# Zain-Jiang/Dict-TTS

Measured on AMD Instinct MI355X. Metric: mel-frames/sec, end-to-end text->mel->wav (audio-samples/sec = 256x; RTF reported alongside), higher is better.
Workload: dtype f16 (vocoder ResBlocks fp16 MFMA, serial convolutions bf16 hi/lo split; acoustic model fp32-grade: fp32 MFMA / bf16 three-piece operands x 6 products)

## Files before the change

dict_tts_amd/csrc/context.hip:

```cpp
#include "ctx.h"

using namespace dtts;

constexpr int TUNE_RELEASE_MASK = (1 << 8) | (1 << 9) | (1 << 12) | (1 << 13) | (1 << 14) | (1 << 15);

static std::string g_create_err;

namespace dtts {

int fail(dtts_ctx* h, int code, const char* fmt, ...) {
    char buf[512];
    va_list ap;
    va_start(ap, fmt);
    vsnprintf(buf, sizeof buf, fmt, ap);
    va_end(ap);
    if (h) h->err = buf;
    else g_create_err = buf;
    return code;
}

}

extern "C" {

int dtts_config_sizeof(void) { return (int)sizeof(dtts_config); }

void dtts_default_config(dtts_config* c) {
    memset(c, 0, sizeof *c);
    c->hidden_size = 192;
    c->num_heads = 2;
    c->enc_ffn_kernel_size = 5;
    c->enc_layers = 4;
    c->gloss_dim = 768;
    c->word_size = 8000;
    c->value_embedding_size = 185;
    c->n_phone = 6;
    c->audio_num_mel_bins = 80;
    c->latent_size = 16;
    c->fvae_enc_dec_hidden = 192;
    c->fvae_kernel_size = 5;
    c->fvae_dec_n_layers = 4;
    c->fvae_enc_n_layers = 8;
    c->prior_glow_hidden = 64;
    c->glow_kernel_size = 3;
    c->prior_glow_n_blocks = 4;
    c->prior_glow_n_layers = 4;
    c->dur_predictor_layers = 3;
    c->dur_predictor_kernel = 5;
    c->dur_chans = 128;
    c->frames_multiple = 4;
    c->language_zh = 1;
    c->upsample_initial_channel = 512;
    c->n_upsamples = 4;
    const int ur[4] = {8, 8, 2, 2}, uk[4] = {16, 16, 4, 4}, rk[3] = {3, 7, 11};
    for (int i = 0; i < 4; ++i) {
        c->upsample_rates[i] = ur[i];
        c->upsample_kernel_sizes[i] = uk[i];
    }
    c->n_resblock_kernels = 3;
    for (int i = 0; i < 3; ++i) {
        c->resblock_kernel_sizes[i] = rk[i];
        c->resblock_dilation_sizes[i][0] = 1;
        c->resblock_dilation_sizes[i][1] = 3;
        c->resblock_dilation_sizes[i][2] = 5;
    }
    c->vocoder_precision = DTTS_VOC_F16;
    c->fft_layers = 4;
    c->fft_kernel_size = 9;
    c->fft_use_pos_embed = 1;
    c->fft_use_last_norm = 1;
}

int dtts_create(const dtts_config* cfg, dtts_handle* out) {
    if (!cfg || !out) return fail(nullptr, DTTS_E_INVAL, "dtts_create: null argument");
    if (cfg->tune_flags & ~TUNE_RELEASE_MASK)
        return fail(nullptr, DTTS_E_INVAL, "dtts_create: tune_flags 0x%x carries bits this library does not honour (supported mask 0x%x)",
                    (unsigned)cfg->tune_flags, (unsigned)TUNE_RELEASE_MASK);
    if (cfg->n_resblock_kernels >= 0 && cfg->n_resblock_kernels <= 4) {
        int two = 0;
        for (int j = 0; j < cfg->n_resblock_kernels; ++j) {
            const int32_t* d = cfg->resblock_dilation_sizes[j];
            if (d[0] < 1 || d[1] < 1 || d[2] < 0)
                return fail(nullptr, DTTS_E_INVAL, "dtts_create: resblock_dilation_sizes[%d] = (%d, %d, %d): the first two dilations must be >= 1, the third >= 1 (ResBlock1) or 0 (ResBlock2)",
                            j, (int)d[0], (int)d[1], (int)d[2]);
            two += d[2] == 0 ? 1 : 0;
        }
        if (two != 0 && two != cfg->n_resblock_kernels)
            return fail(nullptr, DTTS_E_INVAL, "dtts_create: resblock_dilation_sizes mixes two-dilation (ResBlock2, third entry 0) and three-dilation (ResBlock1) rows: "
                        "%d of %d rows have a third entry of 0", two, (int)cfg->n_resblock_kernels);
    }
    int ndev = 0;
    if (hipGetDeviceCount(&ndev) != hipSuccess || ndev == 0)
        return fail(nullptr, DTTS_E_HIP, "dtts_create: no HIP device visible (the HIP path has no CPU fallback)");
    if (cfg->hidden_size % 64 || cfg->hidden_size / cfg->num_heads > 96 || cfg->gloss_dim > 768 || cfg->gloss_dim % 4 ||
        cfg->n_upsamples > 8 || cfg->n_resblock_kernels > 4 || cfg->latent_size % 8 || cfg->prior_glow_hidden % 32 ||
        cfg->fvae_enc_dec_hidden % 32)
        return fail(nullptr, DTTS_E_INVAL, "dtts_create: unsupported configuration");
    dtts_ctx* h = new dtts_ctx();
    h->cfg = *cfg;
    h->tune = cfg->tune_flags;
    {
        static unsigned long long instance = 0;
        int dev = 0;
        (void)hipGetDevice(&dev);
        unsigned long long z = (unsigned long long)time(nullptr) * 0x9E3779B97F4A7C15ull ^ ((unsigned long long)getpid() << 32) ^
                               ((unsigned long long)dev << 20) ^ ++instance;
        z = (z ^ (z >> 30)) * 0xBF58476D1CE4E5B9ull;
        z = (z ^ (z >> 27)) * 0x94D049BB133111EBull;
        h->noise_seed = z ^ (z >> 31);
    }
    h->guard_on = cfg->vocoder_range_guard != 0;
    h->resblock2 = cfg->n_resblock_kernels > 0 && cfg->resblock_dilation_sizes[0][2] == 0;
    (void)hipGetDevice(&h->device);
    if (hipDeviceGetAttribute(&h->n_cu, hipDeviceAttributeMultiprocessorCount, h->device) != hipSuccess || h->n_cu <= 0) h->n_cu = 256;
    h->debug_rz = cfg->debug_redzone != 0;
    h->a_fft.debug = h->a_enc.debug = h->a_dec.debug = h->a_voc.debug = h->a_spk.debug = h->a_post.debug = h->debug_rz;
    *out = h;
    return DTTS_OK;
}

void dtts_destroy(dtts_handle h) {
    if (h && h->bad_host) {
        (void)hipDeviceSynchronize();
        (void)hipHostFree((void*)h->bad_host);
        h->bad_host = nullptr;
    }
    if (!h) return;
    (void)hipDeviceSynchronize();
    for (void* p : h->allocs) (void)hipFree(p);
    if (h->amax_bits) (void)hipFree(h->amax_bits);
    h->a_fft.release();
    h->a_enc.release();
    h->a_dec.release();
    h->a_voc.release();
    h->a_spk.release();
    h->a_post.release();
    for (auto& t : h->timers)
        for (auto e : t.pool) (void)hipEventDestroy(e);
    delete h;
}

const char* dtts_last_error(dtts_handle h) { return h ? h->err.c_str() : g_create_err.c_str(); }

int dtts_load_weight(dtts_handle h, const char* name, const void* host_ptr, const int64_t* shape, int ndim, int dtype) {
    if (!h || !name || !host_ptr || ndim < 0 || ndim > 8) return fail(h, DTTS_E_INVAL, "dtts_load_weight: bad argument");
    if (dtype != DTTS_F32) return fail(h, DTTS_E_INVAL, "dtts_load_weight(%s): only fp32 tensors are accepted", name);
    HostTensor t;
    t.shape.assign(shape, shape + ndim);
    const int64_t n = t.numel();
    t.f.assign((const float*)host_ptr, (const float*)host_ptr + n);
    h->w[name] = std::move(t);
    return DTTS_OK;
}

int dtts_finalize_weights(dtts_handle h, int parts) {
    if (!h) return DTTS_E_INVAL;
    h->err.clear();
    int rc = DTTS_OK;
    if ((parts & DTTS_PART_ACOUSTIC) && !h->acoustic_ready) rc = build_acoustic(h);
    if (rc == DTTS_OK && (parts & DTTS_PART_VOCODER) && !h->vocoder_ready) rc = build_vocoder(h);
    if (rc == DTTS_OK && (parts & DTTS_PART_FFT) && !h->fft_ready) rc = build_fft(h);
    if (rc == DTTS_OK) {
        for (auto it = h->w.begin(); it != h->w.end();) {
            const bool a = it->first.rfind("model.", 0) == 0 && h->acoustic_ready;
            const bool v = it->first.rfind("vocoder.", 0) == 0 && h->vocoder_ready;
            const bool f = it->first.rfind("fft.", 0) == 0 && h->fft_ready;
            it = (a || v || f) ? h->w.erase(it) : std::next(it);
        }
    }
    return rc;
}

int dtts_load_weights(dtts_handle h, const char* name, const void* host_ptr, const int64_t* shape, int ndim, int dtype) {
    return dtts_load_weight(h, name, host_ptr, shape, ndim, dtype);
}

int dtts_timer_enable(dtts_handle h, int which) {
    if (!h || which < 1 || which >= DTTS_TIMER_COUNT) return DTTS_E_INVAL;
    h->timers[which].enabled = true;
    return DTTS_OK;
}

static void timer_collect(TimerSlot& t) {
    for (size_t i = 0; i + 1 < t.used; i += 2) {
        float ms = 0;
        if (hipEventElapsedTime(&ms, t.pool[i], t.pool[i + 1]) == hipSuccess) t.ms_done += ms;
    }
    t.used = 0;
}

int dtts_timer_read(dtts_handle h, int which, double* ms_total, int64_t* launches) {
    if (!h || which < 1 || which >= DTTS_TIMER_COUNT) return DTTS_E_INVAL;
    HIPCHK(hipDeviceSynchronize());
    TimerSlot& t = h->timers[which];
    timer_collect(t);
    if (ms_total) *ms_total = t.ms_done;
    if (launches) *launches = t.launches;
    return DTTS_OK;
}

int dtts_timer_reset(dtts_handle h) {
    if (!h) return DTTS_E_INVAL;
    HIPCHK(hipDeviceSynchronize());
    for (auto& t : h->timers) {
        t.used = 0;
        t.ms_done = 0;
        t.launches = 0;
    }
    return DTTS_OK;
}

namespace {
struct RzZone { const unsigned char* p; unsigned n; unsigned id; };
__global__ void redzone_check_kernel(const RzZone* z, int nz, unsigned long long* out) {
    const RzZone q = z[blockIdx.x];
    unsigned bad = 0;
    for (unsigned i = threadIdx.x; i < q.n; i += blockDim.x) bad += q.p[i] != 0xFF ? 1u : 0u;
    if (bad) {
        atomicAdd(out, (unsigned long long)bad);
        atomicMin(out + 1, (unsigned long long)q.id);
    }
}
}

int dtts_debug_poke(dtts_handle h, dtts_stream stream) {
    if (!h) return DTTS_E_INVAL;
    if (!h->debug_rz) return fail(h, DTTS_E_STATE, "dtts_debug_poke: the context was not created with dtts_config.debug_redzone = 1");
    char* target = nullptr;
    for (Arena* a : {&h->a_voc, &h->a_enc, &h->a_dec, &h->a_fft, &h->a_spk, &h->a_post})
        if (!target && a->base && !a->bufs.empty()) target = a->base + a->bufs[0].start + a->bufs[0].bytes;
    if (!target && !h->rz_static.empty()) target = h->rz_static[0].p + h->rz_static[0].bytes;
    if (!target) return fail(h, DTTS_E_STATE, "dtts_debug_poke: nothing allocated yet");
    HIPCHK(hipMemsetAsync(target, 0, 1, (hipStream_t)stream));
    return DTTS_OK;
}

int dtts_debug_check(dtts_handle h, int64_t* damaged_bytes, dtts_stream stream) {
    if (!h || !damaged_bytes) return DTTS_E_INVAL;
    *damaged_bytes = -1;
    if (!h->debug_rz) return fail(h, DTTS_E_STATE, "dtts_debug_check: the context was not created with dtts_config.debug_redzone = 1");
    hipStream_t s = (hipStream_t)stream;
    HIPCHK(hipStreamSynchronize(s));
    std::vector<RzZone> zones;
    std::vector<std::string> names;
    auto zone = [&](const char* p0, size_t n, const std::string& name) {
        if (!n) return;
        zones.push_back({(const unsigned char*)p0, (unsigned)n, (unsigned)names.size()});
        names.push_back(name);
    };
    const std::pair<const char*, Arena*> arenas[] = {{"encode workspace", &h->a_enc}, {"decode workspace", &h->a_dec}, {"vocoder workspace", &h->a_voc}, {"fft workspace", &h->a_fft}, {"speaker workspace", &h->a_spk}, {"posterior workspace", &h->a_post}};
    for (const auto& a : arenas) {
        const auto& bufs = a.second->bufs;
        const char* base = a.second->base;
        for (size_t i = 0; i < bufs.size(); ++i) {
            const std::string me = std::string(a.first) + " buffer #" + std::to_string(i) + " (" + std::to_string(bufs[i].bytes) + " B)";
            const size_t end = bufs[i].start + bufs[i].bytes, padded_end = bufs[i].start + ((bufs[i].bytes + 255) & ~(size_t)255);
            zone(base + bufs[i].start - RZ, RZ, i ? "AFTER " + std::string(a.first) + " buffer #" + std::to_string(i - 1) + " / BEFORE " + me : "BEFORE " + me);
            zone(base + end, padded_end - end, "AFTER " + me + " (alignment slack)");
            if (i + 1 == bufs.size()) zone(base + padded_end, std::min(RZ, a.second->cap - padded_end), "AFTER " + me);
        }
    }
    for (size_t i = 0; i < h->rz_static.size(); ++i) {
        const auto& b = h->rz_static[i];
        const size_t padded = (b.bytes + 255) & ~(size_t)255;
        const std::string me = "weight pack / table #" + std::to_string(i) + " (" + std::to_string(b.bytes) + " B)";
        zone(b.p - RZ, RZ, "BEFORE " + me);
        zone(b.p + b.bytes, padded + RZ - b.bytes, "AFTER " + me);
    }
    if (zones.empty()) {
        *damaged_bytes = 0;
        return DTTS_OK;
    }
    RzZone* dz = nullptr;
    unsigned long long* dout = nullptr;
    unsigned long long hout[2] = {0ull, ~0ull};
    HIPCHK(hipMalloc((void**)&dz, zones.size() * sizeof(RzZone)));
    hipError_t e = hipMalloc((void**)&dout, sizeof hout);
    if (e == hipSuccess) e = hipMemcpy(dz, zones.data(), zones.size() * sizeof(RzZone), hipMemcpyHostToDevice);
    if (e == hipSuccess) e = hipMemcpy(dout, hout, sizeof hout, hipMemcpyHostToDevice);
    if (e == hipSuccess) {
        hipLaunchKernelGGL(redzone_check_kernel, dim3((unsigned)zones.size()), dim3(256), 0, s, dz, (int)zones.size(), dout);
        e = hipGetLastError();
    }
    if (e == hipSuccess) e = hipStreamSynchronize(s);
    if (e == hipSuccess) e = hipMemcpy(hout, dout, sizeof hout, hipMemcpyDeviceToHost);
    (void)hipFree(dz);
    if (dout) (void)hipFree(dout);
    if (e != hipSuccess) return fail(h, DTTS_E_HIP, "dtts_debug_check: %s", hipGetErrorString(e));
    *damaged_bytes = (int64_t)hout[0];
    if (hout[0]) h->err = "red zone damaged: " + std::to_string(hout[0]) + " bytes in " + std::to_string(zones.size()) + " zones; first: " +
                          (hout[1] < names.size() ? names[hout[1]] : std::string("?"));
    return DTTS_OK;
}

}
```

dict_tts_amd/csrc/ctx.h:

```cpp
#pragma once
#include <hip/hip_runtime.h>

#include <algorithm>
#include <climits>
#include <cmath>
#include <cstdarg>
#include <cstdio>
#include <cstring>
#include <cstdlib>
#include <ctime>
#include <functional>
#include <unistd.h>
#include <map>
#include <string>
#include <vector>

#include "../../include/dicttts_hip.h"
#include "conv1d.h"
#include "ops.h"
#include "vconv.h"
#include "rblock.h"
#include "vpair.h"
#include "rb2x.h"
#include "flowstack.h"

#define DTTS_TUNE(h, bit) (((h)->tune & (bit)) != 0)

namespace dtts {

struct HostTensor {
    std::vector<float> f;
    std::vector<int64_t> shape;
    int64_t numel() const {
        int64_t n = 1;
        for (auto s : shape) n *= s;
        return n;
    }
};

constexpr size_t RZ = 4096;

struct Arena {
    char* base = nullptr;
    size_t cap = 0, off = 0;
    bool debug = false;
    struct Buf { size_t start, bytes; };
    std::vector<Buf> bufs;
    static constexpr int DBG_BUFS = 1024;
    hipError_t reserve(size_t n, hipStream_t s) {
        off = 0;
        bufs.clear();
        if (debug) n += (size_t)DBG_BUFS * (RZ + 256);
        if (n > cap) {
            if (base) {
                hipError_t e = hipDeviceSynchronize();
                if (e != hipSuccess) return e;
                (void)hipFree(base);
                base = nullptr;
                cap = 0;
            }
            n = n + n / 8 + (1 << 20);
            hipError_t e = hipMalloc((void**)&base, n);
            if (e != hipSuccess) return e;
            cap = n;
        }
        if (debug) return hipMemsetAsync(base, 0xFF, cap, s);
        return hipSuccess;
    }
    void rewind() {
        off = 0;
        bufs.clear();
    }
    template <class T>
    T* alloc(size_t count) {
        if (debug) off += RZ;
        size_t bytes = (count * sizeof(T) + 255) & ~(size_t)255;
        if (off + bytes + (debug ? RZ : 0) > cap) return nullptr;
        T* p = (T*)(base + off);
        if (debug) bufs.push_back({off, count * sizeof(T)});
        off += bytes;
        return p;
    }
    void release() {
        if (base) (void)hipFree(base);
        base = nullptr;
        cap = off = 0;
        bufs.clear();
    }
};

struct EncLayer {
    PackedConv qkv, o, ffn1, ffn2;
    float *g1 = nullptr, *b1 = nullptr, *g2 = nullptr, *b2 = nullptr;
};
struct Encoder {
    std::vector<EncLayer> l;
    float *lg = nullptr, *lb = nullptr;
};
struct WNet {
    PackedConv cond;
    std::vector<PackedConv> in, rs;
    int hidden = 0, layers = 0;
};
struct Flow {
    PackedConv pre, post;
    WNet wn;
    int in_coff = 0, out_coff = 0;
};

struct TimerSlot {
    bool enabled = false;
    std::vector<hipEvent_t> pool;
    size_t used = 0;
    double ms_done = 0;
    int64_t launches = 0;
};

}

struct dtts_ctx {
    dtts_config cfg;
    std::string err;
    std::map<std::string, dtts::HostTensor> w;
    std::vector<void*> allocs;
    bool debug_rz = false;
    int device = 0;
    int n_cu = 256;
    struct StaticBuf { char* p; size_t bytes; };
    std::vector<StaticBuf> rz_static;
    bool acoustic_ready = false, vocoder_ready = false, fft_ready = false;
    std::vector<dtts::EncLayer> fft;
    float *fft_g = nullptr, *fft_b = nullptr, *fft_alpha = nullptr;
    dtts::Arena a_fft;
    float *word_emb = nullptr, *pinyin_emb = nullptr;
    dtts::Encoder sem, lin;
    dtts::PackedConv s2_q, s2_kT, s2_k, s2_v, s2_o;
    std::vector<dtts::PackedConv> dur_conv;
    std::vector<float*> dur_g, dur_b;
    float *dur_w = nullptr, *dur_bias = nullptr;
    dtts::PackedConv g_pre, g_pre_poly, dec_pre, dec_out;
    std::vector<dtts::Flow> flows;
    float* fs_w = nullptr;
    dtts::PackedConv fs_cond;
    dtts::WNet dec_wn;
    dtts::PackedConv conv_pre, conv_post;
    std::vector<dtts::PackedConv> ups;
    std::vector<std::vector<dtts::PackedConv>> rb1, rb2;
    std::vector<std::vector<dtts::PackedConv>> rbf1, rbf2;
    bool resblock2 = false;
    int hop = 1;
    int tune = 0;
    float *post_w = nullptr, *post_b = nullptr;
    dtts::Arena a_enc, a_dec, a_voc;
    unsigned* amax_bits = nullptr;
    unsigned long long noise_counter = 0x5EEDull;
    unsigned long long noise_seed = 0;
    unsigned long long* ovf_dev = nullptr;
    bool guard_on = false;
    unsigned* bad_dev = nullptr;
    volatile unsigned* bad_host = nullptr;
    double wc_lin = 0, wc_const = 0, est_lin = 0, est_const = 0;
    bool voc_span = false;
    int amax_cap = 0;
    int B = 0, T_w = 0, L_k = 0, P = 0, T_mel = 0;
    bool encoded = false;
    float *weo = nullptr, *dur = nullptr, *pron_attn = nullptr, *dict_attn = nullptr, *context = nullptr, *x_mask = nullptr;
    int64_t* m2w = nullptr;
    int *mel_lens = nullptr, *lens = nullptr;
    dtts::TimerSlot timers[DTTS_TIMER_COUNT];
    int t_entries = 0;
    int *t_off = nullptr, *t_poff = nullptr, *t_pmmax = nullptr;
    float *t_keys = nullptr, *t_values = nullptr, *t_key_map = nullptr;
    int64_t *t_pinyin = nullptr, *t_pinyin_map = nullptr;
    int spk_kind = 0;
    int spk_n = 0;
    float *spk_w = nullptr, *spk_bias = nullptr;
    dtts::Arena a_spk;
    float* spk_rows = nullptr;
    unsigned long long* spk_flag = nullptr;
    int spk_armed_B = 0;
    unsigned spk_gen = 0, enc_spk_gen = 0;
    bool enc_spk = false;
    bool post_ready = false;
    std::string post_missing, post_unsupported;
    dtts::PackedConv post_pre;
    dtts::WNet post_wn;
    float *post_wt = nullptr, *post_bias = nullptr;
    std::vector<dtts::Flow> flows_fwd;
    float* fs_w_fwd = nullptr;
    dtts::PackedConv fs_cond_fwd;
    dtts::Arena a_post;
};

namespace dtts {

int fail(dtts_ctx* h, int code, const char* fmt, ...);

#define HIPCHK(expr)                                                                                       \
    do {                                                                                                   \
        hipError_t _e = (expr);                                                                            \
        if (_e != hipSuccess) return fail(h, DTTS_E_HIP, "%s failed: %s", #expr, hipGetErrorString(_e));   \
    } while (0)

#define LAUNCH(expr)                                                                                          \
    do {                                                                                                      \
        hipError_t _e = (expr);                                                                               \
        if (_e != hipSuccess) return fail(h, DTTS_E_HIP, "%s: %s", #expr, hipGetErrorString(_e));             \
    } while (0)

void* dev_alloc(dtts_ctx* h, size_t bytes);
void dev_free(dtts_ctx* h, void* user);

template <class T>
T* upload(dtts_ctx* h, const std::vector<T>& v) {
    T* d = (T*)dev_alloc(h, v.size() * sizeof(T));
    if (!d) return nullptr;
    if (!v.empty() && hipMemcpy(d, v.data(), v.size() * sizeof(T), hipMemcpyHostToDevice) != hipSuccess) return nullptr;
    return d;
}

bool pack_conv(dtts_ctx* h, PackedConv& L, int engine, int C_out, int C_in, int K, const std::function<float(int, int, int)>& getw,
               const std::vector<float>& bias, int dil, int stride, int pad, int gate_H = 0, double flops_per_row = -1, int frag = 32);

struct Need {
    dtts_ctx* h;
    std::string missing;
    const HostTensor* get(const std::string& name) {
        auto it = h->w.find(name);
        if (it == h->w.end()) {
            if (missing.empty()) missing = name;
            return nullptr;
        }
        return &it->second;
    }
};

const HostTensor* folded_weight(dtts_ctx* h, Need& need, const std::string& base);
std::vector<float> bias_of(Need& need, const std::string& base);
bool pack_plain(dtts_ctx* h, Need& need, PackedConv& L, int engine, const std::string& base, int dil, int stride, int pad,
                bool with_bias = true, int gate_H = 0, int frag = 32);
bool pack_transposed(dtts_ctx* h, Need& need, PackedConv& L, int engine, const std::string& base, int u, int p);
float* upload_named(dtts_ctx* h, Need& need, const std::string& name);

ConvParams base_params(const float* x, int ldx, int B, int T_in, int T_out, float* y, int ldy);
void set_res(ConvParams& p, int s, const float* res, int ld);
VConvParams vparams(const PackedConv& L, const unsigned short* x, const int* lens, int B, int T);
VConvParams vparams_x3(const PackedConv& L, const float* xf, int ld, float in_slope, const int* lens, int B, int T);

struct Timed {
    dtts_ctx* h;
    int which;
    hipStream_t s;
    hipEvent_t e1 = nullptr;
    Timed(dtts_ctx* h_, int which_, hipStream_t s_) : h(h_), which(which_), s(s_) {
        TimerSlot& t = h->timers[which];
        if (!t.enabled) return;
        if (which == DTTS_TIMER_VOC_CONV && h->voc_span) {
            t.launches += 1;
            return;
        }
        if (t.used + 2 > t.pool.size()) {
            for (int i = 0; i < 256; ++i) {
                hipEvent_t e;
                if (hipEventCreate(&e) != hipSuccess) return;
                t.pool.push_back(e);
            }
        }
        hipEvent_t e0 = t.pool[t.used];
        e1 = t.pool[t.used + 1];
        t.used += 2;
        t.launches += 1;
        (void)hipEventRecord(e0, s);
    }
    void stop() {
        if (e1) (void)hipEventRecord(e1, s);
        e1 = nullptr;
    }
    ~Timed() { stop(); }
};

int build_acoustic(dtts_ctx* h);
int build_vocoder(dtts_ctx* h);
int build_fft(dtts_ctx* h);

}
```

dict_tts_amd/csrc/rb_common.h:

```cpp
#pragma once
#include <hip/hip_runtime.h>
#include <stdint.h>
#include "voc_el.h"

namespace dtts {

constexpr int VP_ST_AUX = 18;
constexpr int VP_LD_AUX = 18;
constexpr int VP_XI_AUX = 2;
constexpr int RB_X_AUX = 0;

typedef __attribute__((ext_vector_type(8))) __bf16 bf16x8;
typedef __attribute__((ext_vector_type(16))) float f32x16;
typedef __attribute__((ext_vector_type(4))) float f32x4;

__device__ __forceinline__ unsigned rf2bf(float f) {
    const __bf16 h = (__bf16)f;
    return (unsigned)__builtin_bit_cast(unsigned short, h);
}

typedef __attribute__((ext_vector_type(2))) float f32x2_t;
typedef __attribute__((ext_vector_type(2))) __bf16 bf16x2_t;
__device__ __forceinline__ unsigned pack2bf(float a, float b) {
    const bf16x2_t v = __builtin_convertvector(f32x2_t{a, b}, bf16x2_t);
    return __builtin_bit_cast(unsigned, v);
}
__device__ __forceinline__ float lrelu(float a, float slope) {
    float r;
    const float b = a * slope;
    asm("v_max_f32 %0, %1, %2" : "=v"(r) : "v"(a), "v"(b));
    return r;
}

typedef __attribute__((ext_vector_type(8))) _Float16 f16x8;
typedef __attribute__((ext_vector_type(2))) _Float16 f16x2_t;

template <int EL>
__device__ __forceinline__ unsigned pack2(float a, float b) {
    if constexpr (EL == EL_F16) {
        const f16x2_t v = __builtin_convertvector(f32x2_t{a, b}, f16x2_t);
        return __builtin_bit_cast(unsigned, v);
    } else {
        return pack2bf(a, b);
    }
}
template <int EL>
__device__ __forceinline__ float lrelu_op(float a, float slope) {
    if constexpr (EL == EL_F16) return __builtin_amdgcn_fmed3f(a, a * slope, 65504.f);
    else return lrelu(a, slope);
}
template <int EL>
__device__ __forceinline__ uint2 act4(const f32x4& v, float slope) {
    const f32x2_t a = {v[0], v[1]}, b = {v[2], v[3]};
    const f32x2_t ta = a * slope, tb = b * slope;
    if constexpr (EL == EL_F16) {
        const _Float16 hs = (_Float16)slope;
        const f16x2_t slope2 = {hs, hs};
        const f16x2_t ha = __builtin_convertvector(a, f16x2_t), hb = __builtin_convertvector(b, f16x2_t);
        const f16x2_t ra = __builtin_elementwise_max(ha, ha * slope2), rb = __builtin_elementwise_max(hb, hb * slope2);
        (void)ta;
        (void)tb;
        return make_uint2(__builtin_bit_cast(unsigned, ra), __builtin_bit_cast(unsigned, rb));
    } else {
        float r0, r1, r2, r3;
        asm("v_max_f32 %0, %1, %2" : "=v"(r0) : "v"(a[0]), "v"(ta[0]));
        asm("v_max_f32 %0, %1, %2" : "=v"(r1) : "v"(a[1]), "v"(ta[1]));
        asm("v_max_f32 %0, %1, %2" : "=v"(r2) : "v"(b[0]), "v"(tb[0]));
        asm("v_max_f32 %0, %1, %2" : "=v"(r3) : "v"(b[1]), "v"(tb[1]));
        return make_uint2(pack2<EL>(r0, r1), pack2<EL>(r2, r3));
    }
}

__device__ __forceinline__ int ovf4(const f32x4& v, float slope) {
    int n = 0;
#pragma unroll
    for (int e = 0; e < 4; ++e) n += (__builtin_fabsf(v[e]) > 65504.f) ? 1 : 0;
    return n;
}

template <int EL>
__device__ __forceinline__ f32x16 mfma16(const uint4& a, const uint4& b, const f32x16& c) {
    if constexpr (EL == EL_F16)
        return __builtin_amdgcn_mfma_f32_32x32x16_f16(__builtin_bit_cast(f16x8, a), __builtin_bit_cast(f16x8, b), c, 0, 0, 0);
    else
        return __builtin_amdgcn_mfma_f32_32x32x16_bf16(__builtin_bit_cast(bf16x8, a), __builtin_bit_cast(bf16x8, b), c, 0, 0, 0);
}

template <int M>
struct MfmaShape;

template <>
struct MfmaShape<32> {
    static constexpr int FRAG = 32;
    static constexpr int CI = 16;
    static constexpr int KB = 32;
    static constexpr int WF = 1;
    static constexpr int XF = 1;
    static constexpr int XROWS = 32;
    static constexpr int RD = 4;
    static constexpr int QB = 1;
    typedef f32x16 acc_t;
    static __device__ __forceinline__ int row(int lane, int qi) { return lane & 31; }
    static __device__ __forceinline__ int chan(int lane, int qi) { return 8 * qi + 4 * (lane >> 5); }
    static __device__ __forceinline__ int xoff(int lane, int pitch) { return (lane & 31) * pitch + (lane >> 5) * 16; }
    static __device__ __forceinline__ f32x4 quad(const acc_t& a, int qi) { return f32x4{a[4 * qi], a[4 * qi + 1], a[4 * qi + 2], a[4 * qi + 3]}; }
    static __device__ __forceinline__ void set_quad(acc_t& a, int qi, const f32x4& v) {
#pragma unroll
        for (int e = 0; e < 4; ++e) a[4 * qi + e] = v[e];
    }
    template <int EL>
    static __device__ __forceinline__ void mma(acc_t& d, const uint4* w, const uint4* const (&x)[XF], const acc_t& c) {
        d = mfma16<EL>(w[0], *x[0], c);
    }
};

template <>
struct MfmaShape<16> {
    static constexpr int FRAG = 16;
    static constexpr int CI = 32;
    static constexpr int KB = 64;
    static constexpr int WF = 2;
    static constexpr int XF = 2;
    static constexpr int XROWS = 16;
    static constexpr int QB = 2;
    static constexpr int RD = 2;
    struct acc_t {
        f32x4 q[4];
    };
    static __device__ __forceinline__ int row(int lane, int qi) { return 16 * (qi & 1) + (lane & 15); }
    static __device__ __forceinline__ int chan(int lane, int qi) { return 16 * (qi >> 1) + 4 * (lane >> 4); }
    static __device__ __forceinline__ int xoff(int lane, int pitch) { return (lane & 15) * pitch + (lane >> 4) * 16; }
    static __device__ __forceinline__ f32x4 quad(const acc_t& a, int qi) { return a.q[qi]; }
    static __device__ __forceinline__ void set_quad(acc_t& a, int qi, const f32x4& v) { a.q[qi] = v; }
    template <int EL>
    static __device__ __forceinline__ void mma(acc_t& d, const uint4* w, const uint4* const (&x)[XF], const acc_t& c) {
#pragma unroll
        for (int ch = 0; ch < 2; ++ch)
#pragma unroll
            for (int rh = 0; rh < 2; ++rh) {
                if constexpr (EL == EL_F16)
                    d.q[2 * ch + rh] = __builtin_amdgcn_mfma_f32_16x16x32_f16(__builtin_bit_cast(f16x8, w[ch]), __builtin_bit_cast(f16x8, *x[rh]), c.q[2 * ch + rh], 0, 0, 0);
                else
                    d.q[2 * ch + rh] = __builtin_amdgcn_mfma_f32_16x16x32_bf16(__builtin_bit_cast(bf16x8, w[ch]), __builtin_bit_cast(bf16x8, *x[rh]), c.q[2 * ch + rh], 0, 0, 0);
            }
    }
};

constexpr int RB_GUARD = 40;

template <int NTW, int RD>
__device__ __forceinline__ void rb_preload(uint4 (&ring)[RD][NTW], const uint4* w, int kg_stride) {
#pragma unroll
    for (int s = 0; s < RD - 1; ++s)
#pragma unroll
        for (int n = 0; n < NTW; ++n) ring[s][n] = w[(size_t)s * kg_stride + n * 64];
}

template <int EL, int MT, int NT, int NKG, int PITCH, bool CINIT, int MH = 1, class SH = MfmaShape<32>>
__device__ __forceinline__ void rb_group(typename SH::acc_t (&acc)[MH * MT][NT], const typename SH::acc_t (&cinit)[NT], uint4 (&ring)[SH::RD][NT * SH::WF],
                                         uint4 (&xa)[MT], const char* act, const uint4* wpf, int xb, int dilP, int g) {
    constexpr int GPT = (NKG >= 4) ? NKG / 4 : 1;
    constexpr int KGS = NKG * SH::CI * 2 * SH::WF;
    constexpr int HSTRIDE = MT * 32 * PITCH;
    constexpr int RD = SH::RD, WF = SH::WF, KB = SH::KB;
    static_assert(4 % RD == 0, "a group of 4 steps is whole turns of the ring");
#pragma unroll
    for (int u = 0; u < 4; ++u) {
#pragma unroll
        for (int h = 0; h < MH; ++h) {
            if (h == 0) {
#pragma unroll
                for (int n = 0; n < NT * WF; ++n) ring[(u + RD - 1) % RD][n] = wpf[u * KGS + n * 64];
            }
            constexpr int NP = MT * SH::XF;
            int cur = 0;
            if constexpr (SH::XF > 1) {
                if constexpr (NKG >= 4) cur = xb + ((g * 4 + u) % NKG) * KB + h * HSTRIDE;
                else cur = xb + (u / NKG) * dilP + (u % NKG) * KB + h * HSTRIDE;
            }
            int off;
            if (h + 1 < MH) {
                if constexpr (NKG >= 4) off = xb + ((g * 4 + u) % NKG) * KB + (h + 1) * HSTRIDE;
                else off = xb + (u / NKG) * dilP + (u % NKG) * KB + (h + 1) * HSTRIDE;
            } else if constexpr (NKG >= 4) {
                const int kgn = (g * 4 + u + 1);
                off = (u == 3 && g == GPT - 1) ? xb + dilP : xb + (kgn % NKG) * KB;
            } else {
                const int un = u + 1;
                off = xb + (un / NKG) * dilP + (un % NKG) * KB;
            }
            __builtin_amdgcn_sched_barrier(0);
#pragma unroll
            for (int m = 0; m < MT; ++m)
#pragma unroll
                for (int n = 0; n < NT; ++n) {
                    const uint4* xf[SH::XF];
#pragma unroll
                    for (int f = 0; f < SH::XF; ++f) xf[f] = &xa[(m * SH::XF + f) % MT];
                    if (CINIT && u == 0) SH::template mma<EL>(acc[h * MT + m][n], &ring[u % RD][n * WF], xf, cinit[n]);
                    else SH::template mma<EL>(acc[h * MT + m][n], &ring[u % RD][n * WF], xf, acc[h * MT + m][n]);
                    if (n == NT - 1) {
                        __builtin_amdgcn_sched_barrier(0);
#pragma unroll
                        for (int f = 0; f < SH::XF; ++f) {
                            const int p = m * SH::XF + f, pn = (p + MT) % NP;
                            xa[p % MT] = *(const uint4*)(act + (p + MT < NP ? cur : off) + (pn / SH::XF * 32 + pn % SH::XF * SH::XROWS) * PITCH);
                        }
                        __builtin_amdgcn_sched_barrier(0);
                    }
                }
            __builtin_amdgcn_sched_barrier(0);
        }
    }
}

template <int EL, int MT, int NT, int NKG, int PITCH, bool CINIT = false, int MH = 1, class SH = MfmaShape<32>>
__device__ __forceinline__ void rb_contract(typename SH::acc_t (&acc)[MH * MT][NT], uint4 (&ring)[SH::RD][NT * SH::WF], const char* act, int xrow0,
                                            const uint4* w, int S, int dilP, const typename SH::acc_t (*cinit)[NT] = nullptr) {
    typedef typename SH::acc_t acc_t;
    constexpr int TU = (NKG >= 4) ? 1 : 4 / NKG;
    constexpr int GPT = (NKG >= 4) ? NKG / 4 : 1;
    constexpr int KGS = NKG * SH::CI * 2 * SH::WF;
    uint4 xa[MT];
#pragma unroll
    for (int p = 0; p < MT; ++p) xa[p] = *(const uint4*)(act + xrow0 + (p / SH::XF * 32 + p % SH::XF * SH::XROWS) * PITCH);
    const uint4* wpf = w + (SH::RD - 1) * KGS;
    int xb = xrow0;
    int g = 0;
    int s0 = 0;
    if constexpr (CINIT) {
        if (SH::FRAG == 16 || S > 0) {
            rb_group<EL, MT, NT, NKG, PITCH, true, MH, SH>(acc, *cinit, ring, xa, act, wpf, xb, dilP, 0);
            s0 = 4;
            wpf += 4 * KGS;
            if constexpr (NKG >= 4) {
                if (++g == GPT) {
                    g = 0;
                    xb += dilP;
                }
            } else {
                xb += TU * dilP;
            }
        } else {
#pragma unroll
            for (int m = 0; m < MH * MT; ++m)
#pragma unroll
                for (int n = 0; n < NT; ++n) acc[m][n] = (*cinit)[n];
        }
    }
    for (; s0 < S; s0 += 4) {
        const acc_t(&dummy)[NT] = *(const acc_t(*)[NT])acc[0];
        rb_group<EL, MT, NT, NKG, PITCH, false, MH, SH>(acc, dummy, ring, xa, act, wpf, xb, dilP, g);
        wpf += 4 * KGS;
        if constexpr (NKG >= 4) {
            if (++g == GPT) {
                g = 0;
                xb += dilP;
            }
        } else {
            xb += TU * dilP;
        }
    }
}

template <int NT, int RD>
__device__ __forceinline__ void rb2_preload(uint4 (&ring)[RD][NT], const uint4* w, int kgs) {
#pragma unroll
    for (int s = 0; s < RD - 1; ++s)
#pragma unroll
        for (int n = 0; n < NT; ++n) ring[s][n] = w[(size_t)s * kgs + n * 64];
}

template <int EL, int MT, int NT, int NKG, int PITCH, int RD, bool FIRST, bool CINIT>
__device__ __forceinline__ bool rb2_group(f32x16 (&acc)[MT][NT], const f32x16 (&cinit)[NT], uint4 (&ring)[RD][NT], uint4 (&xa)[MT],
                                          const char* act, const uint4* wpf, int xb, int dilP, int left) {
    constexpr int KGS = (NKG / 2) * 64;
    static_assert(RD % NKG == 0 && RD % 2 == 0, "a ring turn covers whole taps");
#pragma unroll
    for (int u = 0; u < RD; ++u) {
        if (u && u % NKG == 0 && u >= left) return true;
#pragma unroll
        for (int n = 0; n < NT; ++n) ring[(u + RD - 1) % RD][n] = wpf[u * KGS + n * 64];
        const int off = xb + ((u + 1) / NKG) * dilP + ((u + 1) % NKG) * 32;
        __builtin_amdgcn_sched_barrier(0);
#pragma unroll
        for (int m = 0; m < MT; ++m)
#pragma unroll
            for (int n = 0; n < NT; ++n) {
                if (FIRST && CINIT && u == 0) acc[m][n] = mfma16<EL>(ring[u][n], xa[m], cinit[n]);
                else acc[m][n] = mfma16<EL>(ring[u][n], xa[m], acc[m][n]);
                if (n == NT - 1) {
                    __builtin_amdgcn_sched_barrier(0);
                    xa[m] = *(const uint4*)(act + off + m * 32 * PITCH);
                    __builtin_amdgcn_sched_barrier(0);
                }
            }
        __builtin_amdgcn_sched_barrier(0);
    }
    return left <= RD;
}

template <int EL, int MT, int NT, int NKG, int PITCH, int RD, bool CINIT>
__device__ __forceinline__ void rb2_contract(f32x16 (&acc)[MT][NT], uint4 (&ring)[RD][NT], const char* act, int xrow0, const uint4* w, int S,
                                             int dilP, const f32x16 (&cinit)[NT]) {
    constexpr int KGS = (NKG / 2) * 64;
    uint4 xa[MT];
#pragma unroll
    for (int m = 0; m < MT; ++m) xa[m] = *(const uint4*)(act + xrow0 + m * 32 * PITCH);
    const uint4* wpf = w + (RD - 1) * KGS;
    int xb = xrow0;
    if (rb2_group<EL, MT, NT, NKG, PITCH, RD, true, CINIT>(acc, cinit, ring, xa, act, wpf, xb, dilP, S)) return;
    for (int left = S - RD;; left -= RD) {
        wpf += RD * KGS;
        xb += (RD / NKG) * dilP;
        if (rb2_group<EL, MT, NT, NKG, PITCH, RD, false, CINIT>(acc, cinit, ring, xa, act, wpf, xb, dilP, left)) return;
    }
}

}
```

dict_tts_amd/csrc/rblock.h:

```cpp
#pragma once
#include <hip/hip_runtime.h>
#include <stdint.h>
#include "voc_el.h"

namespace dtts {

struct RBlockParams {
    const float* x;
    float* S;
    unsigned short* Sa;
    struct Set {
        const uint4* w1[3];
        const uint4* w2[3];
        const float* b1[3];
        const float* b2[3];
        int dil[3];
        int K, Kp;
    } rb[3];
    int nrb;
    const int* lens;
    int B, T;
    int K;
    int mode;
    int last_mode;
    int drop_S;
    float div, slope;
    float* wav;
    const float* post_w;
    const float* post_b;
    int el;
    unsigned* tile_ctr;
    int pre_off;
    unsigned* bad;
    unsigned long long* ovf;
    int small_tile;
    int : 32;
    int s_private;
};

__host__ __device__ inline int rblock_halo_of(int K, const int* dil) {
    const int need = (K - 1) / 2 * (dil[0] + dil[1] + dil[2] + 3);
    return need > 6 * (K - 1) ? need : 6 * (K - 1);
}
__host__ __device__ inline int rblock_halo(const RBlockParams& p) {
    int h = 6 * (p.K - 1);
    for (int j = 0; j < p.nrb && j < 3; ++j) {
        const int need = rblock_halo_of(p.rb[j].K, p.rb[j].dil);
        h = need > h ? need : h;
    }
    return h;
}

bool rblock_supported(int C, int K);
int rblock_padded_taps(int C, int K);
hipError_t rblock_launch(const RBlockParams& p, int C, hipStream_t stream);
long long rblock_private_rows(int C, int halo, int B, int T);
int rblock_stage_tile_rows(int C, int halo);
bool rblock_stage_launch_fits(int C, int halo, int B, bool wav);

}
```

dict_tts_amd/csrc/rblock.hip:

```cpp
#include "rblock.h"
#include "rb_common.h"

#include <algorithm>
#include <type_traits>
#include <cstdlib>

namespace dtts {

#ifdef RB_STAMP
__device__ unsigned long long rb_stamps[2][12][16];
extern "C" __attribute__((visibility("default"))) int dtts_debug_rb_stamps(unsigned long long* host, int reset) {
    hipError_t e = hipMemcpyFromSymbol(host, HIP_SYMBOL(rb_stamps), sizeof(rb_stamps));
    if (e == hipSuccess && reset) {
        static unsigned long long z[2][12][16];
        e = hipMemcpyToSymbol(HIP_SYMBOL(rb_stamps), z, sizeof z);
    }
    return (int)e;
}
#define RB_T(k) do { const unsigned long long _n = __builtin_amdgcn_s_memrealtime(); tq[k] += _n - t_last; t_last = _n; } while (0)
#else
#define RB_T(k)
#endif

template <int C, int MT, int NT, int WT, int WC, int EL, int PS, bool GUARD, bool TB = false>
__global__ __launch_bounds__(64 * WT * WC, (64 * WT * WC <= 256) ? 2 : 1) void rblock_kernel(const RBlockParams p) {
    static_assert(WC * NT * 32 == C, "channel tiling must cover C");
    extern __shared__ __attribute__((aligned(16))) char smem[];
    constexpr int THREADS = 64 * WT * WC;
    constexpr int W = 32 * MT * WT;
    constexpr int PITCH = C * 2 + 16;
    constexpr int NKG = C / 16;
    constexpr int EP = C * 4 + 16;
    constexpr int F4 = C / 4, SROWS = WT * 32;
    constexpr size_t ACT_BYTES = (size_t)(W + 2 * RB_GUARD) * PITCH;
    char* act = smem;
    char* act2 = TB ? smem + ACT_BYTES : smem;
    char* stage = TB ? act2 + RB_GUARD * PITCH : smem + ACT_BYTES;

    int tid = threadIdx.x, lane = tid & 63, wave = tid >> 6;
    int wt = wave % WT, wc = wave / WT;
    const int H = rblock_halo(p);
    const int TT = W - 2 * H;
    constexpr int PK = 7, PH = (PK - 1) / 2;
    const int TTo = p.wav ? TT - 2 * PH : TT;

    int* pre = (int*)(smem + p.pre_off);
    auto zero_guard_bands = [&](int t) {
        for (int idx = t; idx < 2 * RB_GUARD * (PITCH / 16); idx += THREADS) {
            const int r = idx / (PITCH / 16), c = idx % (PITCH / 16);
            const int row = r < RB_GUARD ? r : W + r;
            *(uint4*)(act + row * PITCH + c * 16) = make_uint4(0, 0, 0, 0);
            if constexpr (TB) *(uint4*)(act2 + row * PITCH + c * 16) = make_uint4(0, 0, 0, 0);
        }
    };
    zero_guard_bands(tid);
    int total = 0, j = blockIdx.x;
    if constexpr (PS) {
        for (int i = tid; i < p.B; i += THREADS) {
            const int l = p.lens ? p.lens[i] : p.T;
            pre[p.B + 1 + i] = (l + TTo - 1) / TTo;
            pre[2 * p.B + 1 + i] = l;
        }
        __syncthreads();
        for (int i = tid; i <= p.B; i += THREADS) {
            int a = 0;
            for (int u = 0; u < i; ++u) a += pre[p.B + 1 + u];
            pre[i] = a;
        }
        __syncthreads();
        total = pre[p.B];
        if (j >= total) return;
    }
    const int G = gridDim.x;

    typedef __attribute__((ext_vector_type(4))) unsigned int u32x4;
    constexpr int RPP = THREADS / F4;
    constexpr int PER = SROWS / RPP;
    static_assert(THREADS % F4 == 0 && SROWS % RPP == 0, "row-coalesced staging");
    int c4 = tid % F4, r0 = tid / F4;
    auto tile_row = [&](int m, int u) { const int sr = r0 + RPP * u; return ((sr >> 5) * MT + m) * 32 + (sr & 31); };

    auto locate = [&](int jj, int& bb) {
        while (pre[bb + 1] <= jj) ++bb;
        bb = __builtin_amdgcn_readfirstlane(bb);
    };
    auto load_x = [&](f32x16 (&d)[NT], int m, int bb, int base, int ln) {
        const auto rs = __builtin_amdgcn_make_buffer_rsrc((void*)(p.x + (long long)bb * p.T * C), 0, ln * C * 4, 0x00020000);
        const int o0 = ((base + wt * MT * 32 + (lane & 31)) * C + wc * NT * 32 + 4 * (lane >> 5)) * 4;
#pragma unroll
        for (int n = 0; n < NT; ++n)
#pragma unroll
            for (int q = 0; q < 4; ++q) {
                const u32x4 v = __builtin_amdgcn_raw_buffer_load_b128(rs, o0 + (m * 32 * C + n * 32 + 8 * q) * 4, 0, RB_X_AUX);
                const f32x4 f = __builtin_bit_cast(f32x4, v);
#pragma unroll
                for (int e = 0; e < 4; ++e) d[n][4 * q + e] = f[e];
            }
    };
    auto len_of = [&](int bb) { return __builtin_amdgcn_readfirstlane(pre[2 * p.B + 1 + bb]); };

    int b = 0, len, t0;
    if constexpr (PS) {
        locate(j, b);
        len = len_of(b);
        t0 = (j - pre[b]) * TTo - (p.wav ? PH : 0);
    } else {
        b = blockIdx.y;
        len = __builtin_amdgcn_readfirstlane(p.lens ? p.lens[b] : p.T);
        t0 = blockIdx.x * TTo - (p.wav ? PH : 0);
        if (t0 + (p.wav ? PH : 0) >= len) return;
    }
    f32x16 xr[MT][NT];
    if constexpr (PS) {
#pragma unroll
        for (int m = 0; m < MT; ++m) load_x(xr[m], m, b, t0 - H, len);
    } else {
        const auto rs_x = __builtin_amdgcn_make_buffer_rsrc((void*)(p.x + (long long)b * p.T * C), 0, len * C * 4, 0x00020000);
        const int g0 = ((t0 - H + r0) * C + c4 * 4) * 4;
        u32x4 ld[MT][PER] = {};
#pragma unroll
        for (int m = 0; m < MT; ++m)
#pragma unroll
            for (int u = 0; u < PER; ++u) ld[m][u] = __builtin_amdgcn_raw_buffer_load_b128(rs_x, g0 + (tile_row(m, u) - r0) * (C * 4), 0, RB_X_AUX);
#pragma unroll
        for (int m = 0; m < MT; ++m) {
            if (m) __syncthreads();
#pragma unroll
            for (int u = 0; u < PER; ++u) *(u32x4*)(stage + (r0 + RPP * u) * EP + c4 * 16) = ld[m][u];
            __syncthreads();
#pragma unroll
            for (int n = 0; n < NT; ++n)
#pragma unroll
                for (int q = 0; q < 4; ++q) {
                    const f32x4 v = *(const f32x4*)(stage + (wt * 32 + (lane & 31)) * EP + ((wc * NT + n) * 32 + 8 * q + 4 * (lane >> 5)) * 4);
#pragma unroll
                    for (int e = 0; e < 4; ++e) xr[m][n][4 * q + e] = v[e];
                }
        }
    }

    const int kg_stride = (C / 32) * 64;
    int r = 0;

#ifdef RB_STAMP
    unsigned long long tq[16] = {0, 0, 0, 0, 0, 0, 0, 0, 0, 0, 0, 0, 0, 0, 0, 0};
    unsigned long long t_last = __builtin_amdgcn_s_memrealtime();
#endif
#pragma unroll 1
    for (;;) {
    if constexpr (PS) {
        tid = threadIdx.x;
        asm volatile("" : "+v"(tid));
        lane = tid & 63, wave = __builtin_amdgcn_readfirstlane(tid >> 6);
        wt = wave % WT, wc = wave / WT;
        c4 = tid % F4, r0 = tid / F4;
    }
    const int xlane = (RB_GUARD + wt * MT * 32 + (lane & 31)) * PITCH + (lane >> 5) * 16;
    const size_t wlane = (size_t)(wc * NT) * 64 + lane;
    if constexpr (PS) r = __builtin_amdgcn_readfirstlane(r);
    else r = 0;
    const RBlockParams::Set& R = p.rb[PS ? r : 0];
    const int Kr = R.K;
    constexpr bool REAL_STEPS = (NKG < 4);
    const int S = (REAL_STEPS ? Kr : R.Kp) * NKG;
    const bool last_rb = !PS || r + 1 == p.nrb;
    const int mode = (!PS || p.nrb == 1 || r == 0) ? p.mode : (last_rb ? p.last_mode : 1);
    const bool wav_now = p.wav && last_rb;
    t0 = __builtin_amdgcn_readfirstlane(t0);
    const int base_t = t0 - H;
    const long long brow = (long long)b * p.T;
    unsigned claim = 0;
    if (PS && p.tile_ctr && tid == 0 && last_rb) claim = atomicAdd(p.tile_ctr, 1u);
    int jn = j + G;
    bool has_next = PS && jn < total;
    int bn = b, lenn = len, t0n = 0;
    auto plan_next = [&]() {
        if (!last_rb) {
            has_next = true;
            jn = j;
            bn = b;
            lenn = len;
            t0n = t0;
            return;
        }
        has_next = PS && jn < total;
        bn = b;
        if (has_next) {
            locate(jn, bn);
            lenn = len_of(bn);
            t0n = (jn - pre[bn]) * TTo - (p.wav ? PH : 0);
        }
    };
    if (!(PS && p.tile_ctr) || !last_rb) plan_next();
    const auto rs_s = p.s_private ? __builtin_amdgcn_make_buffer_rsrc((void*)p.S, 0, p.s_private, 0x00020000)
                                  : __builtin_amdgcn_make_buffer_rsrc((void*)(p.S + brow * C), 0, len * C * 4, 0x00020000);

    auto load_bias = [&](f32x4 (&bb)[NT][4], const float* bias) {
#pragma unroll
        for (int n = 0; n < NT; ++n)
#pragma unroll
            for (int q = 0; q < 4; ++q) bb[n][q] = *(const f32x4*)(bias + (wc * NT + n) * 32 + 8 * q + 4 * (lane >> 5));
    };
    const bool all_inb = base_t >= 0 && base_t + W <= len;
    int n_ovf = 0;
    auto write_act_impl = [&](char* dst, const f32x16 (&v)[MT][NT], auto masked_tag) {
        constexpr bool MASKED = decltype(masked_tag)::value;
#pragma unroll
        for (int m = 0; m < MT; ++m) {
            const int row = (wt * MT + m) * 32 + (lane & 31);
            const int t = base_t + row;
            const bool inb = !MASKED || (t >= 0 && t < len);
            const bool counted = inb && row >= H && row < H + TT;
#pragma unroll
            for (int n = 0; n < NT; ++n)
#pragma unroll
                for (int q = 0; q < 4; ++q) {
                    const int co = (wc * NT + n) * 32 + 8 * q + 4 * (lane >> 5);
                    f32x4 v4 = {v[m][n][4 * q], v[m][n][4 * q + 1], v[m][n][4 * q + 2], v[m][n][4 * q + 3]};
                    uint2 pk = act4<EL>(v4, 0.1f);
                    if constexpr (GUARD) n_ovf += counted ? ovf4(v4, 0.1f) : 0;
                    if constexpr (MASKED) {
                        if (!inb) pk = make_uint2(0, 0);
                    }
                    *(uint2*)(dst + (RB_GUARD + row) * PITCH + co * 2) = pk;
                }
        }
    };
    auto write_act = [&](char* dst, const f32x16 (&v)[MT][NT]) {
        if (all_inb) write_act_impl(dst, v, std::false_type{});
        else write_act_impl(dst, v, std::true_type{});
    };

    uint4 ring[4][NT];
    f32x4 bb[NT][4];
    RB_T(10);
    rb_preload<NT>(ring, R.w1[0] + wlane, kg_stride);
    load_bias(bb, R.b1[0]);
    write_act(act, xr);
    RB_T(0);
    __syncthreads();
    RB_T(1);

    f32x16 acc[MT][NT];
#pragma unroll 1
    for (int it = 0; it < 3; ++it) {
        f32x16 cinit[NT];
#pragma unroll
        for (int n = 0; n < NT; ++n)
#pragma unroll
            for (int q = 0; q < 4; ++q)
#pragma unroll
                for (int e = 0; e < 4; ++e) cinit[n][4 * q + e] = bb[n][q][e];
        load_bias(bb, R.b2[it]);
        const int d = R.dil[it];
        if constexpr (REAL_STEPS) {
            if (S) rb2_contract<EL, MT, NT, NKG, PITCH, 4, true>(acc, ring, act, xlane - ((Kr - 1) / 2) * d * PITCH, R.w1[it] + wlane, S, d * PITCH, cinit);
            else rb_contract<EL, MT, NT, NKG, PITCH, true, 1>(acc, ring, act, 0, R.w1[it] + wlane, 0, 0, &cinit);
        } else
            rb_contract<EL, MT, NT, NKG, PITCH, true, 1>(acc, ring, act, xlane - ((Kr - 1) / 2) * d * PITCH, R.w1[it] + wlane, S, d * PITCH, &cinit);
        rb_preload<NT>(ring, R.w2[it] + wlane, kg_stride);
        RB_T(2);
        if constexpr (!TB) __syncthreads();
        RB_T(3);
        write_act(act2, acc);
        RB_T(4);
        __syncthreads();
        RB_T(5);
#pragma unroll
        for (int m = 0; m < MT; ++m)
#pragma unroll
            for (int n = 0; n < NT; ++n)
#pragma unroll
                for (int q = 0; q < 4; ++q)
#pragma unroll
                    for (int e = 0; e < 4; ++e) xr[m][n][4 * q + e] += bb[n][q][e];
        if (it < 2) load_bias(bb, R.b1[it + 1]);
        if constexpr (REAL_STEPS) {
            if (S) rb2_contract<EL, MT, NT, NKG, PITCH, 4, false>(xr, ring, act2, xlane - ((Kr - 1) / 2) * PITCH, R.w2[it] + wlane, S, PITCH, cinit);
        } else
            rb_contract<EL, MT, NT, NKG, PITCH, false, 1>(xr, ring, act2, xlane - ((Kr - 1) / 2) * PITCH, R.w2[it] + wlane, S, PITCH);
        if (it < 2) rb_preload<NT>(ring, R.w1[it + 1] + wlane, kg_stride);
        if (PS && p.tile_ctr && last_rb && it == 2 && tid == 0) pre[3 * p.B + 1] = G + (int)claim;
        RB_T(6);
        if (!TB || it == 2) __syncthreads();
        RB_T(7);
        if (it < 2) {
            write_act(act, xr);
            RB_T(0);
            __syncthreads();
            RB_T(1);
        }
    }

    if (PS && p.tile_ctr && last_rb) {
        jn = __builtin_amdgcn_readfirstlane(pre[3 * p.B + 1]);
        plan_next();
    }
    {
    const auto rs_a = __builtin_amdgcn_make_buffer_rsrc((void*)(p.Sa ? p.Sa + brow * C : (unsigned short*)(p.S + brow * C)), 0,
                                                        len * C * 2, 0x00020000);
    constexpr int CW = NT * 32, F4W = CW / 4, RPI = 64 / F4W, NRD = 32 / RPI;
    const int er = lane / F4W, ec = lane % F4W;
    const int goffw = (p.s_private ? (j * TT - H) * C : base_t * C) * 4 + (wc * CW + ec * 4) * 4;
    static_assert(F4W == 8 && RPI == 8 && NRD == 4, "the conflict-free row order below is for 8 lanes per row, 8 rows per access");
    const int erow_slab_base = C == 32 ? er : (er >> 2) + ((er & 1) ? 16 : 0) + ((er & 2) ? 8 : 0);
    auto srow = [&](int u) { return (C == 32 ? 8 : 2) * u + erow_slab_base; };
    auto erow = [&](int m, int u) { return (wt * MT + m) * 32 + srow(u); };
    auto eoff = [&](int m, int u) {
        const int row = erow(m, u);
        return (row >= H && row < H + TT) ? goffw + row * (C * 4) : (int)0x80000000;
    };
    u32x4 sold[MT][NRD];
#pragma unroll
    for (int m = 0; m < MT; ++m)
#pragma unroll
        for (int u = 0; u < NRD; ++u) {
            sold[m][u] = u32x4{0u, 0u, 0u, 0u};
            if (mode >= 1) sold[m][u] = p.nrb > 1 ? __builtin_amdgcn_raw_buffer_load_b128(rs_s, eoff(m, u), 0, 0)
                                                  : __builtin_amdgcn_raw_buffer_load_b128(rs_s, eoff(m, u), 0, VP_LD_AUX);
        }
    RB_T(12);
    constexpr int OP = C * 4;
    char* otile = smem;
    char* estage = wav_now ? smem + ((TB || (size_t)TT * OP > ACT_BYTES) ? (size_t)TT * OP : ACT_BYTES) : stage;
    char* stg = estage + (wt * 32) * EP + (wc * CW) * 4;
#pragma unroll
    for (int m = 0; m < MT; ++m) {
#pragma unroll
        for (int n = 0; n < NT; ++n)
#pragma unroll
            for (int q = 0; q < 4; ++q) {
                f32x4 v;
#pragma unroll
                for (int e = 0; e < 4; ++e) v[e] = xr[m][n][4 * q + e];
                *(f32x4*)(stg + (lane & 31) * EP + (n * 32 + 8 * q + 4 * (lane >> 5)) * 4) = v;
            }
        if (has_next) load_x(xr[m], m, bn, t0n - H, lenn);
        __builtin_amdgcn_fence(__ATOMIC_RELEASE, "wavefront");
        __builtin_amdgcn_wave_barrier();
        __builtin_amdgcn_fence(__ATOMIC_ACQUIRE, "wavefront");
        RB_T(13);
#pragma unroll
        for (int u = 0; u < NRD; ++u) {
            const int off = eoff(m, u);
            f32x4 o = *(const f32x4*)(stg + srow(u) * EP + ec * 16);
            o += __builtin_bit_cast(f32x4, sold[m][u]);
            if (wav_now) {
                const int row = erow(m, u);
                if (row >= H && row < H + TT) {
                    const int t = base_t + row;
#pragma unroll
                    for (int e = 0; e < 4; ++e) o[e] = (t >= 0 && t < len) ? lrelu(o[e] / p.div, p.slope) : 0.f;
                    *(f32x4*)(otile + (size_t)(row - H) * OP + (wc * CW + ec * 4) * 4) = o;
                }
                continue;
            }
            if (mode == 2) {
#pragma unroll
                for (int e = 0; e < 4; ++e) o[e] = o[e] / p.div;
            }
            if (!(mode == 2 && p.Sa && p.drop_S)) {
                if (p.nrb > 1 && !last_rb) __builtin_amdgcn_raw_buffer_store_b128(__builtin_bit_cast(u32x4, o), rs_s, off, 0, 0);
                else __builtin_amdgcn_raw_buffer_store_b128(__builtin_bit_cast(u32x4, o), rs_s, off, 0, VP_ST_AUX);
            }
            if (mode == 2 && p.Sa) {
                typedef __attribute__((ext_vector_type(2))) unsigned int u32x2;
                const u32x2 pk = {pack2bf(lrelu(o[0], p.slope), lrelu(o[1], p.slope)), pack2bf(lrelu(o[2], p.slope), lrelu(o[3], p.slope))};
                __builtin_amdgcn_raw_buffer_store_b64(pk, rs_a, off == (int)0x80000000 ? off : off >> 1, 0, VP_ST_AUX);
            }
        }
        __builtin_amdgcn_fence(__ATOMIC_RELEASE, "wavefront");
        __builtin_amdgcn_wave_barrier();
        __builtin_amdgcn_fence(__ATOMIC_ACQUIRE, "wavefront");
        RB_T(14);
    }
    if constexpr (C == 32) if (wav_now) {
        __syncthreads();
        const int q8 = tid & 7, rr = tid >> 3;
        f32x4 wq[PK];
#pragma unroll
        for (int k = 0; k < PK; ++k) wq[k] = *(const f32x4*)(p.post_w + k * C + q8 * 4);
        const float pb = p.post_b[0];
        float* wb = p.wav + brow;
        constexpr int PR = 3;
        for (int o0 = 0; o0 < TTo; o0 += (THREADS / 8) * PR) {
            const int ob = o0 + rr * PR;
            float a[PR];
#pragma unroll
            for (int i = 0; i < PR; ++i) a[i] = 0.f;
            if (ob < TTo) {
#pragma unroll
                for (int j = 0; j < PR + PK - 1; ++j) {
                    const int row = ob + j < TTo + PK - 1 ? ob + j : TTo + PK - 2;
                    const f32x4 v = *(const f32x4*)(otile + (size_t)row * OP + q8 * 16);
#pragma unroll
                    for (int i = 0; i < PR; ++i) {
                        const int k = j - i;
                        if (k >= 0 && k < PK) {
                            const float d = __builtin_fmaf(v[3], wq[k][3], __builtin_fmaf(v[2], wq[k][2], __builtin_fmaf(v[1], wq[k][1], __fmul_rn(v[0], wq[k][0]))));
                            a[i] = __fadd_rn(a[i], d);
                        }
                    }
                }
            }
#pragma unroll
            for (int i = 0; i < PR; ++i) {
                a[i] += __shfl_xor(a[i], 1, 64);
                a[i] += __shfl_xor(a[i], 2, 64);
                a[i] += __shfl_xor(a[i], 4, 64);
            }
            float pre[PR], th[PR];
            int nf = 0;
#pragma unroll
            for (int i = 0; i < PR; ++i) {
                pre[i] = a[i] + pb;
                th[i] = __builtin_fmaf(-2.f, __builtin_amdgcn_rcpf(__fadd_rn(__builtin_amdgcn_exp2f(pre[i] * 2.885390081777927f), 1.f)), 1.f);
            }
            if (q8 == 0) {
#pragma unroll
                for (int i = 0; i < PR; ++i) {
                    const int o = ob + i, t = t0 + PH + o;
                    const bool nonfin = !(__builtin_fabsf(pre[i]) <= 3.0e38f);
                    if (o < TTo && t < len) {
                        wb[t] = nonfin ? __builtin_nanf("") : th[i];
                        nf += nonfin ? 1 : 0;
                    }
                }
                if (nf && p.bad) atomicAdd(p.bad, (unsigned)nf);
            }
        }
    }
    }
    RB_T(8);
#ifdef RB_STAMP
    tq[11] += 1;
#endif
    if constexpr (GUARD) {
        if (n_ovf) atomicAdd(p.ovf, (unsigned long long)n_ovf);
    }
    if (!has_next) break;
    r = last_rb ? 0 : r + 1;
    if (wav_now) {
        __syncthreads();
        zero_guard_bands(threadIdx.x);
    }
    j = jn;
    b = bn;
    len = lenn;
    t0 = t0n;
    }
#ifdef RB_STAMP
    {
        const int w = threadIdx.x >> 6;
        if ((threadIdx.x & 63) == 0 && (w == 0 || w == WT * WC - 1)) {
            const int slot = (C == 32 ? 0 : C == 64 ? 1 : C == 128 ? 2 : 3) * 3 + (p.K == 3 ? 0 : p.K == 7 ? 1 : 2);
            for (int k = 0; k < 16; ++k) atomicAdd(&rb_stamps[w == 0 ? 0 : 1][slot][k], tq[k]);
        }
    }
#endif
}

template <int C, int MT, int WT, bool TB>
static size_t rb_lds_bytes(int TT, bool wav) {
    constexpr int W = 32 * MT * WT, PITCH = C * 2 + 16, EP = C * 4 + 16;
    constexpr size_t ACT = (size_t)(W + 2 * RB_GUARD) * PITCH;
    if (wav)
        return TB ? std::max(2 * ACT, (size_t)TT * C * 4 + (size_t)WT * 32 * EP) : std::max((size_t)TT * C * 4, ACT) + (size_t)WT * 32 * EP;
    return TB ? std::max(2 * ACT, ACT + (size_t)RB_GUARD * PITCH + (size_t)WT * 32 * EP) : ACT + (size_t)WT * 32 * EP;
}
static size_t rb_table_bytes(int B) { return (size_t)(3 * B + 2) * sizeof(int); }

template <int C, int MT, int NT, int WT, int WC, int EL, int PS, bool GUARD = false, bool TB = false>
static hipError_t rb_launch_cfg(const RBlockParams& p, hipStream_t stream) {
    constexpr int W = 32 * MT * WT;
    const int H = rblock_halo(p), TT = W - 2 * H;
    if (TT < 32) return hipErrorInvalidValue;
    if ((long long)p.T * C * 4 >= (1LL << 31)) return hipErrorInvalidValue;
    if (p.wav && (C != 32 || (p.nrb == 1 && p.mode != 2) || !p.post_w || !p.post_b)) return hipErrorInvalidValue;
    size_t lds = rb_lds_bytes<C, MT, WT, TB>(TT, p.wav != nullptr);
    const int TTo = p.wav ? TT - 6 : TT;
    RBlockParams q = p;
    q.pre_off = (int)lds;
    if (PS) lds += rb_table_bytes(p.B);
    if (lds > 160 * 1024) return hipErrorOutOfMemory;
    if constexpr (EL == EL_F16 && !GUARD) {
        if (p.ovf) return rb_launch_cfg<C, MT, NT, WT, WC, EL, PS, true, TB>(p, stream);
    }
    auto kern = rblock_kernel<C, MT, NT, WT, WC, EL, PS, GUARD, TB>;
    static bool configured_dev[64] = {};
    int cur_dev = 0;
    (void)hipGetDevice(&cur_dev);
    bool& configured = configured_dev[cur_dev & 63];
    if (!configured) {
        hipError_t e = hipFuncSetAttribute((const void*)kern, hipFuncAttributeMaxDynamicSharedMemorySize, 160 * 1024);
        if (e != hipSuccess) return e;
        configured = true;
    }
    constexpr int THREADS = 64 * WT * WC;
    if (!PS) {
        hipLaunchKernelGGL(kern, dim3((p.T + TTo - 1) / TTo, p.B), dim3(THREADS), lds, stream, q);
        return hipGetLastError();
    }
    static int cus_dev[64] = {};
    int& cus = cus_dev[cur_dev & 63];
    if (!cus) {
        hipDeviceProp_t prop;
        if (hipGetDeviceProperties(&prop, cur_dev) != hipSuccess) return hipErrorInvalidDevice;
        cus = prop.multiProcessorCount;
    }
    const int per_cu = std::max(1, std::min({(int)(160 * 1024 / lds), 2048 / THREADS, THREADS <= 256 ? 2 : 1}));
    const long long max_tiles = (long long)p.B * ((p.T + TTo - 1) / TTo);
    const int grid = (int)std::min<long long>((long long)cus * per_cu, max_tiles);
    if (grid <= 0) return hipSuccess;
    hipLaunchKernelGGL(kern, dim3(grid), dim3(THREADS), lds, stream, q);
    return hipGetLastError();
}

bool rblock_supported(int C, int K) {
    if (!(K & 1) || K < 3 || K > 11) return false;
    return C == 32 || C == 64 || ((C == 128 || C == 256) && K == 3);
}

int rblock_stage_tile_rows(int C, int halo) {
    return (C == 32 ? 1024 : 512) - 2 * halo;
}

bool rblock_stage_launch_fits(int C, int halo, int B, bool wav) {
    const int TT = rblock_stage_tile_rows(C, halo);
    if (C != 32 && C != 64) return false;
    const size_t lds = (C == 32 ? rb_lds_bytes<32, 4, 8, false>(TT, wav) : rb_lds_bytes<64, 4, 4, false>(TT, wav)) + rb_table_bytes(B);
    return TT >= 32 && lds <= 160 * 1024;
}

long long rblock_private_rows(int C, int halo, int B, int T) {
    if (C != 32) return 0;
    const int TT = rblock_stage_tile_rows(C, halo), TTo = TT - 6;
    if (TTo < 32) return 0;
    return (long long)B * ((T + TTo - 1) / TTo) * TT;
}

int rblock_padded_taps(int C, int K) {
    const int nkg = C / 16;
    int kp = K;
    while ((kp * nkg) % 4) ++kp;
    return kp;
}

template <int EL>
static hipError_t rb_launch_el(const RBlockParams& p, int C, hipStream_t stream) {
    static int cus_dev[64] = {};
    int cur_dev = 0;
    (void)hipGetDevice(&cur_dev);
    int& cus = cus_dev[cur_dev & 63];
    if (!cus) {
        hipDeviceProp_t prop;
        cus = hipGetDeviceProperties(&prop, cur_dev) == hipSuccess ? prop.multiProcessorCount : 256;
    }
    auto few = [&](int W) {
        const int tt = W - 2 * rblock_halo(p) - (p.wav ? 6 : 0);
        return tt >= 32 && 2 * (long long)p.B * ((p.T + tt - 1) / tt) <= cus;
    };
    if (p.nrb < 1 || p.nrb > 3) return hipErrorInvalidValue;
    if (p.nrb > 1) {
        if (C == 32) return rb_launch_cfg<32, 4, 1, 8, 1, EL, 1>(p, stream);
        if (C == 64) return rb_launch_cfg<64, 4, 1, 4, 2, EL, 1>(p, stream);
        return hipErrorInvalidValue;
    }
#define RB_TRY(call)                                   \
    do {                                               \
        const hipError_t e_ = (call);                  \
        if (e_ != hipErrorOutOfMemory) return e_;      \
    } while (0)
    if (C == 32 && p.K >= 7 && !few(1024)) RB_TRY((rb_launch_cfg<32, 4, 1, 8, 1, EL, 1>(p, stream)));
    if (C == 64 && few(512)) return rb_launch_cfg<64, 4, 1, 2, 2, EL, 1>(p, stream);
    if (C == 128 && few(256)) return rb_launch_cfg<128, 4, 1, 1, 4, EL, 1>(p, stream);
    if (C == 256 && few(128)) return rb_launch_cfg<256, 2, 1, 1, 8, EL, 1>(p, stream);
    if (C == 32) return rb_launch_cfg<32, 4, 1, 4, 1, EL, 0>(p, stream);
    if (C == 64 && p.K >= 7 && !p.small_tile) RB_TRY((rb_launch_cfg<64, 5, 1, 4, 2, EL, 1>(p, stream)));
    if (C == 64) RB_TRY((rb_launch_cfg<64, 4, 1, 4, 2, EL, 1>(p, stream)));
    if (C == 64) return rb_launch_cfg<64, 4, 1, 2, 2, EL, 1>(p, stream);
    if (C == 128) RB_TRY((rb_launch_cfg<128, 4, 1, 2, 4, EL, 1>(p, stream)));
    if (C == 128) return rb_launch_cfg<128, 4, 1, 1, 4, EL, 1>(p, stream);
    if (C == 256) RB_TRY((rb_launch_cfg<256, 4, 1, 1, 8, EL, 1>(p, stream)));
    if (C == 256) return rb_launch_cfg<256, 2, 1, 1, 8, EL, 1>(p, stream);
#undef RB_TRY
    return hipErrorInvalidValue;
}

hipError_t rblock_launch(const RBlockParams& p, int C, hipStream_t stream) {
    return p.el == EL_F16 ? rb_launch_el<EL_F16>(p, C, stream) : rb_launch_el<EL_BF16>(p, C, stream);
}

}
```

dict_tts_amd/csrc/vocoder.hip:

```cpp
#include "ctx.h"

using namespace dtts;

namespace {

bool vocoder_fp16_analysis(dtts_ctx* h, Need& need) {
    const dtts_config& c = h->cfg;
    const std::string v = "vocoder.";
    const int nk = c.n_resblock_kernels;
    std::vector<double> pt_wc[2], pt_m2[2];
    for (int pass = 0; pass < 2; ++pass) {
        const double M = pass;
        auto conv = [&](const std::string& base, const std::vector<double>& uin, const std::vector<double>& min, std::vector<double>& uout,
                        std::vector<double>& mout) -> bool {
            const HostTensor* w = folded_weight(h, need, base);
            const std::vector<float> b = bias_of(need, base);
            if (!w || b.empty() || w->shape.size() != 3) return false;
            const int co_n = (int)w->shape[0], ci_n = (int)w->shape[1], k_n = (int)w->shape[2];
            if ((int)uin.size() < ci_n) return false;
            uout.assign(co_n, 0.0);
            mout.assign(co_n, 0.0);
            for (int co = 0; co < co_n; ++co) {
                double su = std::fabs((double)b[co]), sm = (double)b[co] * b[co];
                for (int ci = 0; ci < ci_n; ++ci) {
                    double a1 = 0, a2 = 0;
                    const float* pw = &w->f[((size_t)co * ci_n + ci) * k_n];
                    for (int k = 0; k < k_n; ++k) {
                        a1 += std::fabs((double)pw[k]);
                        a2 += (double)pw[k] * pw[k];
                    }
                    su += a1 * uin[ci];
                    sm += a2 * min[ci];
                }
                uout[co] = su;
                mout[co] = sm;
            }
            return true;
        };
        std::vector<double> u(c.audio_num_mel_bins, M), m(c.audio_num_mel_bins, M * M), u2, m2;
        if (!conv(v + "conv_pre", u, m, u2, m2)) return false;
        u.swap(u2);
        m.swap(m2);
        for (int i = 0; i < c.n_upsamples; ++i) {
            const int r = c.upsample_rates[i], k_n = c.upsample_kernel_sizes[i], pad = (k_n - r) / 2;
            const HostTensor* w = folded_weight(h, need, v + "ups." + std::to_string(i));
            const std::vector<float> b = bias_of(need, v + "ups." + std::to_string(i));
            if (!w || b.empty() || w->shape.size() != 3 || (int)w->shape[2] != k_n) return false;
            const int ci_n = (int)w->shape[0], co_n = (int)w->shape[1];
            std::vector<double> ux(co_n, 0.0), mx(co_n, 0.0);
            for (int co = 0; co < co_n; ++co)
                for (int ph = 0; ph < r; ++ph) {
                    double su = std::fabs((double)b[co]), sm = (double)b[co] * b[co];
                    for (int ci = 0; ci < ci_n; ++ci) {
                        const float* pw = &w->f[((size_t)ci * co_n + co) * k_n];
                        double a1 = 0, a2 = 0;
                        for (int k = (ph + pad) % r; k < k_n; k += r) {
                            a1 += std::fabs((double)pw[k]);
                            a2 += (double)pw[k] * pw[k];
                        }
                        su += a1 * u[ci];
                        sm += a2 * 0.505 * m[ci];
                    }
                    ux[co] = std::max(ux[co], su);
                    mx[co] = std::max(mx[co], sm);
                }
            std::vector<double> us(co_n, 0.0), ms(co_n, 0.0);
            for (int j = 0; j < nk; ++j) {
                std::vector<double> x = ux, xm = mx, xt, xtm, y, ym, xa(co_n), xam(co_n);
                const std::string rb = v + "resblocks." + std::to_string(i * nk + j);
                for (int mth = 0; mth < (h->resblock2 ? 2 : 3); ++mth) {
                    for (int q = 0; q < co_n; ++q) {
                        pt_wc[pass].push_back(x[q]);
                        pt_m2[pass].push_back(xm[q]);
                        xa[q] = x[q];
                        xam[q] = 0.505 * xm[q];
                    }
                    if (h->resblock2) {
                        if (!conv(rb + ".convs." + std::to_string(mth), xa, xam, y, ym)) return false;
                    } else {
                        if (!conv(rb + ".convs1." + std::to_string(mth), xa, xam, xt, xtm)) return false;
                        for (int q = 0; q < co_n; ++q) {
                            pt_wc[pass].push_back(xt[q]);
                            pt_m2[pass].push_back(xtm[q]);
                            xtm[q] *= 0.505;
                        }
                        if (!conv(rb + ".convs2." + std::to_string(mth), xt, xtm, y, ym)) return false;
                    }
                    for (int q = 0; q < co_n; ++q) {
                        x[q] += y[q];
                        xm[q] += ym[q];
                    }
                }
                for (int q = 0; q < co_n; ++q) {
                    us[q] += x[q] / nk;
                    ms[q] += xm[q] / nk;
                }
            }
            u.swap(us);
            m.swap(ms);
        }
    }
    if (pt_wc[0].size() != pt_wc[1].size()) return false;
    double a_wc = 0, b_wc = 0, a_m2 = 0, b_m2 = 0;
    for (size_t q = 0; q < pt_wc[0].size(); ++q) {
        a_wc = std::max(a_wc, pt_wc[0][q]);
        b_wc = std::max(b_wc, pt_wc[1][q] - pt_wc[0][q]);
        a_m2 = std::max(a_m2, pt_m2[0][q]);
        b_m2 = std::max(b_m2, pt_m2[1][q] - pt_m2[0][q]);
    }
    h->wc_const = a_wc;
    h->wc_lin = b_wc;
    h->est_const = std::sqrt(a_m2);
    h->est_lin = std::sqrt(b_m2);
    return true;
}

bool pack_rb_fused(dtts_ctx* h, Need& need, PackedConv& L, int eng, const std::string& base, int ch, int k, int dil) {
    const HostTensor* w = folded_weight(h, need, base);
    std::vector<float> bias = bias_of(need, base);
    if (!w || bias.empty()) return false;
    const float* pw = w->f.data();
    const int slack = ch >= 64 ? 1 : 2;
    const bool ok = pack_conv(h, L, eng, ch, ch, rblock_padded_taps(ch, k) + slack,
                              [=](int co, int ci, int tap) { return tap < k ? pw[((size_t)co * ch + ci) * k + tap] : 0.f; }, bias, dil, 1, 0);
    L.K = k;
    return ok;
}

bool vpair_pack_fits(const PackedConv& L, int ch, int k) {
    return L.C_in == ch && L.C_out == ch && L.C_in_pad == ch && L.C_out_pad == ch && L.K == k && L.frag == vpair_mfma_shape(ch);
}
bool vpair_runs(const dtts_config& c, bool resblock2, int eng_rb, int ch, int k, int d0, int d1, int d2) {
    const bool fuse = c.vocoder_precision == DTTS_VOC_F16 || !c.vocoder_unfused;
    return fuse && !resblock2 && eng_rb != ENG_BF16X3 && !rblock_supported(ch, k) && vpair_supported(ch, k, d0) && vpair_supported(ch, k, d1) &&
           vpair_supported(ch, k, d2);
}

}

namespace dtts {

int build_vocoder(dtts_ctx* h) {
    Need need{h, ""};
    const dtts_config& c = h->cfg;
    if (c.vocoder_precision != DTTS_VOC_BF16 && c.vocoder_precision != DTTS_VOC_BF16X3 && c.vocoder_precision != DTTS_VOC_F16)
        return fail(h, DTTS_E_INVAL, "vocoder_precision %d is not one of DTTS_VOC_BF16 / _BF16X3 / _F16", c.vocoder_precision);
    if (c.vocoder_precision == DTTS_VOC_F16 && c.audio_num_mel_bins % 4)
        return fail(h, DTTS_E_INVAL, "DTTS_VOC_F16 needs audio_num_mel_bins %% 4 == 0 (got %d); use DTTS_VOC_BF16X3", c.audio_num_mel_bins);
    if (!h->ovf_dev) {
        if (!(h->ovf_dev = (unsigned long long*)dev_alloc(h, sizeof(unsigned long long))) || hipMemset(h->ovf_dev, 0, sizeof(unsigned long long)) != hipSuccess)
            return fail(h, DTTS_E_NOMEM, "range-guard counter");
    }
    if (!h->bad_dev) {
        if (!(h->bad_dev = (unsigned*)dev_alloc(h, sizeof(unsigned))) || hipMemset(h->bad_dev, 0, sizeof(unsigned)) != hipSuccess)
            return fail(h, DTTS_E_NOMEM, "overflow-detector counter");
        void* hp = nullptr;
        if (hipHostMalloc(&hp, 64, hipHostMallocDefault) != hipSuccess) return fail(h, DTTS_E_NOMEM, "overflow-detector host word");
        h->bad_host = (volatile unsigned*)hp;
        *h->bad_host = 0;
    }
    const int eng = c.vocoder_precision == DTTS_VOC_BF16 ? ENG_BF16 : ENG_BF16X3;
    const int eng_rb = c.vocoder_precision == DTTS_VOC_F16 ? ENG_F16 : eng;
    const std::string v = "vocoder.";
    bool ok = pack_plain(h, need, h->conv_pre, eng, v + "conv_pre", 1, 1, 3);
    h->ups.resize(c.n_upsamples);
    h->hop = 1;
    for (int i = 0; ok && i < c.n_upsamples; ++i) {
        const int u = c.upsample_rates[i], k = c.upsample_kernel_sizes[i];
        const bool h2 = c.vocoder_precision == DTTS_VOC_F16 && i == 1 && DTTS_TUNE(h, 8192) && (u * (c.upsample_initial_channel >> (i + 1))) % 256 == 0 &&
                        (c.upsample_initial_channel >> i) % 128 == 0;
        ok = ok && pack_transposed(h, need, h->ups[i], h2 ? ENG_F16 : eng, v + "ups." + std::to_string(i), u, (k - u) / 2);
        h->hop *= u;
    }
    const int nk = c.n_resblock_kernels;
    h->rb1.assign((size_t)c.n_upsamples * nk, {});
    h->rb2.assign((size_t)c.n_upsamples * nk, {});
    const bool rb2x = h->resblock2;
    for (int i = 0; ok && i < c.n_upsamples * nk; ++i) {
        const int j = i % nk, k = c.resblock_kernel_sizes[j], n = rb2x ? 2 : 3;
        const int ch = c.upsample_initial_channel >> (i / nk + 1);
        const std::string r = v + "resblocks." + std::to_string(i);
        const int* dl = c.resblock_dilation_sizes[j];
        const bool vp = vpair_runs(c, rb2x, eng_rb, ch, k, dl[0], dl[1], dl[2]);
        const int frag = vp ? vpair_mfma_shape(ch) : 32;
        h->rb1[i].resize(n);
        if (!rb2x) h->rb2[i].resize(3);
        for (int mth = 0; ok && mth < n; ++mth) {
            const int d = c.resblock_dilation_sizes[j][mth];
            ok = ok && pack_plain(h, need, h->rb1[i][mth], eng_rb, r + (rb2x ? ".convs." : ".convs1.") + std::to_string(mth), d, 1, (k * d - d) / 2, true, 0, frag);
            if (!rb2x) ok = ok && pack_plain(h, need, h->rb2[i][mth], eng_rb, r + ".convs2." + std::to_string(mth), 1, 1, (k - 1) / 2, true, 0, frag);
            if (ok && vp && !vpair_pack_fits(h->rb1[i][mth], ch, k))
                return fail(h, DTTS_E_INVAL, "%s%d: weight shape [%d, %d, %d] is not the configured [%d, %d, %d]", (r + ".convs1.").c_str(), mth, h->rb1[i][mth].C_out,
                            h->rb1[i][mth].C_in, h->rb1[i][mth].K, ch, ch, k);
            if (ok && vp && !vpair_pack_fits(h->rb2[i][mth], ch, k))
                return fail(h, DTTS_E_INVAL, "%s%d: weight shape [%d, %d, %d] is not the configured [%d, %d, %d]", (r + ".convs2.").c_str(), mth, h->rb2[i][mth].C_out,
                            h->rb2[i][mth].C_in, h->rb2[i][mth].K, ch, ch, k);
        }
    }
    h->rbf1.assign((size_t)c.n_upsamples * nk, {});
    h->rbf2.assign((size_t)c.n_upsamples * nk, {});
    for (int i = 0; ok && rb2x && eng_rb != ENG_BF16X3 && i < c.n_upsamples * nk; ++i) {
        const int j = i % nk, k = c.resblock_kernel_sizes[j];
        const int ch = c.upsample_initial_channel >> (i / nk + 1);
        const int d0 = c.resblock_dilation_sizes[j][0], d1 = c.resblock_dilation_sizes[j][1];
        if (!rb2x_supported(ch, k, d0, d1) || h->rb1[i][0].C_in_pad != ch || nk < 2) {
            if (eng_rb == ENG_F16)
                return fail(h, DTTS_E_INVAL, "DTTS_VOC_F16 needs ResBlock2 widths 32/64/128/256, odd kernels 3..11 and a dilation pair whose halo fits the tile "
                            "(resblock %d: %d channels, k=%d, dilations (%d, %d)); use DTTS_VOC_BF16X3", i, ch, k, d0, d1);
            continue;
        }
        h->rbf1[i].resize(2);
        for (int mth = 0; ok && mth < 2; ++mth)
            ok = pack_rb_fused(h, need, h->rbf1[i][mth], eng_rb, v + "resblocks." + std::to_string(i) + ".convs." + std::to_string(mth), ch, k,
                               c.resblock_dilation_sizes[j][mth]);
    }
    for (int i = 0; ok && !rb2x && eng_rb != ENG_BF16X3 && i < c.n_upsamples * nk; ++i) {
        const int j = i % nk, k = c.resblock_kernel_sizes[j];
        const int ch = c.upsample_initial_channel >> (i / nk + 1);
        if (!rblock_supported(ch, k)) {
            const int* dl = c.resblock_dilation_sizes[j];
            if (eng_rb == ENG_F16 && !vpair_runs(c, rb2x, eng_rb, ch, k, dl[0], dl[1], dl[2]))
                return fail(h, DTTS_E_INVAL, "DTTS_VOC_F16 needs ResBlock widths 32/64/128/256 and odd kernels 3..11 (resblock %d: %d channels, k=%d); use DTTS_VOC_BF16X3", i, ch, k);
            continue;
        }
        h->rbf1[i].resize(3);
        h->rbf2[i].resize(3);
        const std::string r = v + "resblocks." + std::to_string(i);
        for (int mth = 0; ok && mth < 3; ++mth) {
            ok = pack_rb_fused(h, need, h->rbf1[i][mth], eng_rb, r + ".convs1." + std::to_string(mth), ch, k, c.resblock_dilation_sizes[j][mth]);
            ok = ok && pack_rb_fused(h, need, h->rbf2[i][mth], eng_rb, r + ".convs2." + std::to_string(mth), ch, k, 1);
        }
    }
    ok = ok && pack_plain(h, need, h->conv_post, eng, v + "conv_post", 1, 1, 3);
    {
        const int last_ch = c.upsample_initial_channel >> c.n_upsamples;
        const HostTensor* w = ok ? folded_weight(h, need, v + "conv_post") : nullptr;
        const std::vector<float> b = ok ? bias_of(need, v + "conv_post") : std::vector<float>();
        bool fusable = ok && eng_rb != ENG_BF16X3 && last_ch == 32 && w && w->shape.size() == 3 && w->shape[0] == 1 && w->shape[1] == 32 &&
                       w->shape[2] == 7 && b.size() == 1 && nk >= 2;
        for (int j = 0; fusable && j < nk; ++j) fusable = !h->rbf1[(size_t)(c.n_upsamples - 1) * nk + j].empty();
        if (fusable) {
            std::vector<float> wt((size_t)7 * 32);
            for (int ci = 0; ci < 32; ++ci)
                for (int k = 0; k < 7; ++k) wt[(size_t)k * 32 + ci] = w->f[(size_t)ci * 7 + k];
            h->post_w = upload(h, wt);
            h->post_b = upload(h, b);
            ok = h->post_w && h->post_b;
        }
    }
    if (!ok) {
        if (!need.missing.empty()) return fail(h, DTTS_E_NOENT, "missing weight tensor '%s'", need.missing.c_str());
        if (h->err.empty()) return fail(h, DTTS_E_NOMEM, "packing / uploading vocoder weights failed");
        return DTTS_E_INVAL;
    }
    if (c.vocoder_precision == DTTS_VOC_F16 && !vocoder_fp16_analysis(h, need)) return fail(h, DTTS_E_NOENT, "fp16 analysis: missing weight tensor '%s'", need.missing.c_str());
    h->vocoder_ready = true;
    return DTTS_OK;
}

}

namespace {

struct StageGeom {
    long long rows[9];
    int ch[9];
    size_t max_elems;
};
StageGeom stage_geom(const dtts_config& c, int B, int T) {
    StageGeom g;
    g.rows[0] = T;
    g.ch[0] = c.upsample_initial_channel;
    g.max_elems = (size_t)B * T * g.ch[0];
    for (int i = 0; i < c.n_upsamples; ++i) {
        g.rows[i + 1] = g.rows[i] * c.upsample_rates[i];
        g.ch[i + 1] = g.ch[i] / 2;
        g.max_elems = std::max<size_t>(g.max_elems, (size_t)B * (size_t)g.rows[i + 1] * (size_t)g.ch[i + 1]);
    }
    return g;
}

struct StageMult { int m[9]; };

__global__ void zero_wav_tails_kernel(float* wav, const int32_t* lens, int T, int hop) {
    const int b = blockIdx.y;
    const long long n = (long long)T * hop;
    int l = lens[b];
    l = l < 0 ? 0 : (l > T ? T : l);
    const long long first = (long long)l * hop;
    const long long i = first + ((long long)blockIdx.x * blockDim.x + threadIdx.x) * 4;
    if (i + 3 < n) *(float4*)(wav + (long long)b * n + i) = make_float4(0.f, 0.f, 0.f, 0.f);
    else for (long long k = i; k < n; ++k) wav[(long long)b * n + k] = 0.f;
}

}

extern "C" __global__ void scale_lens_kernel(const int32_t* lens, int32_t* out, int B, int T, int n_stage, StageMult mult) {
    const int i = blockIdx.x * blockDim.x + threadIdx.x;
    if (i >= B * n_stage) return;
    const int sidx = i / B, b = i % B;
    int l = lens ? lens[b] : T;
    l = l < 0 ? 0 : (l > T ? T : l);
    out[i] = l * mult.m[sidx];
}

namespace {

void scale_lens(const dtts_config& c, const int32_t* lens, int* lensS, int B, int T, hipStream_t s) {
    const int nup = c.n_upsamples;
    StageMult mult;
    mult.m[0] = 1;
    for (int i = 0; i < nup; ++i) mult.m[i + 1] = mult.m[i] * c.upsample_rates[i];
    hipLaunchKernelGGL(scale_lens_kernel, dim3((B * (nup + 1) + 255) / 256), dim3(256), 0, s, lens, lensS, B, T, nup + 1, mult);
}


enum RbPath { RB_WHOLE, RB_VPAIR, RB_CONVS };
RbPath rb_path(const dtts_ctx* h, bool fuse, int ch, size_t rb) {
    if (fuse && !h->rbf1[rb].empty()) return RB_WHOLE;
    if (h->resblock2) return RB_CONVS;
    const auto& c1 = h->rb1[rb];
    return fuse && vpair_runs(h->cfg, false, c1[0].engine, ch, c1[0].K, c1[0].dil, c1[1].dil, c1[2].dil) ? RB_VPAIR : RB_CONVS;
}

struct FusePlan {
    int fuse_n[8];
    size_t s_elems;
};
FusePlan fuse_plan(const dtts_ctx* h, const StageGeom& g, int B, bool fuse) {
    const dtts_config& c = h->cfg;
    const int nup = c.n_upsamples, nk = c.n_resblock_kernels;
    FusePlan pl = {{1, 1, 1, 1, 1, 1, 1, 1}, g.max_elems};
    for (int i = 0; i < nup; ++i) {
        const long long rows = g.rows[i + 1];
        const int ch = g.ch[i + 1];
        if (h->resblock2) continue;
        if (fuse && DTTS_TUNE(h, 4096) && !DTTS_TUNE(h, 512) && nk == 3 && ch == 32 && !h->rbf1[(size_t)i * nk].empty() && !h->rbf1[(size_t)i * nk + 1].empty()) {
            int halo2 = 0;
            for (int j = 0; j < 2; ++j) halo2 = std::max(halo2, rblock_halo_of(h->rbf1[(size_t)i * nk + j][0].K, c.resblock_dilation_sizes[j]));
            const int TT2 = rblock_stage_tile_rows(ch, halo2);
            if (TT2 >= 64 && rblock_stage_launch_fits(ch, halo2, B, false) && (long long)B * ((rows + TT2 - 1) / TT2) >= 2LL * h->n_cu) pl.fuse_n[i] = 2;
            continue;
        }
        bool all = fuse && DTTS_TUNE(h, 512) && nk >= 2 && nk <= 3 && (ch == 32 || ch == 64);
        int halo = 0;
        for (int j = 0; j < nk && all; ++j) {
            all = !h->rbf1[(size_t)i * nk + j].empty();
            if (all) halo = std::max(halo, rblock_halo_of(h->rbf1[(size_t)i * nk + j][0].K, c.resblock_dilation_sizes[j]));
        }
        if (!all) continue;
        const bool with_post = i == nup - 1 && h->post_w;
        const int TT = rblock_stage_tile_rows(ch, halo);
        if (TT < 64 || !rblock_stage_launch_fits(ch, halo, B, with_post) || (long long)B * ((rows + TT - 1) / TT) < 2LL * h->n_cu) continue;
        if (with_post) {
            const long long prow = rblock_private_rows(ch, halo, B, (int)rows);
            if (prow <= 0 || (size_t)prow * ch * sizeof(float) >= (size_t)INT_MAX) continue;
            pl.s_elems = std::max(pl.s_elems, (size_t)prow * ch);
        }
        pl.fuse_n[i] = nk;
    }
    return pl;
}

typedef unsigned short bf;
constexpr int TV = DTTS_TIMER_VOC_CONV;
constexpr int N_CTR = 64;

struct VocRun {
    dtts_ctx* h;
    hipStream_t s;
    int B, nk;
    bool exact;
    int el;
    float* wav;
    float *Xf, *Rf, *Sf, *Rg;
    bf *Xa, *Ra, *Ta, *Sa;
    unsigned* ctrs;
    int n_ctr;
    size_t s_cap_bytes;
    bool post_done;
    int i, ch, Tcur;
    const int* lout;
    bool last_stage;

    template <class P>
    void whole_rb_params(P& rp, int j, int j_last) {
        memset(&rp, 0, sizeof rp);
        rp.x = Xf;
        rp.S = Sf;
        rp.lens = lout;
        rp.B = B;
        rp.T = Tcur;
        rp.mode = j == 0 ? 0 : (j == nk - 1 ? 2 : 1);
        rp.div = (float)nk;
        rp.slope = last_stage ? 0.01f : 0.1f;
        rp.Sa = exact ? nullptr : Sa;
        rp.drop_S = exact ? 0 : 1;
        if (last_stage && j_last == nk - 1 && h->post_w) {
            rp.wav = wav;
            rp.post_w = h->post_w;
            rp.post_b = h->post_b;
            rp.Sa = nullptr;
            post_done = true;
        }
        rp.el = el;
        rp.tile_ctr = n_ctr < N_CTR ? ctrs + n_ctr++ : nullptr;
        rp.ovf = (exact && h->guard_on) ? h->ovf_dev : nullptr;
        rp.bad = h->bad_dev;
    }

    int rblock(int j, int fuse_n) {
        if (nk == 1) return fail(h, DTTS_E_INVAL, "fused ResBlock path needs >= 2 resblock kernels");
        if (j > 0 && j < fuse_n) return DTTS_OK;
        const int j_last = j == 0 ? fuse_n - 1 : j;
        RBlockParams rp;
        whole_rb_params(rp, j, j_last);
        rp.nrb = j_last - j + 1;
        rp.last_mode = j_last == nk - 1 ? 2 : 1;
        for (int jj = j; jj <= j_last; ++jj) {
            RBlockParams::Set& st = rp.rb[jj - j];
            const auto& g1 = h->rbf1[(size_t)i * nk + jj];
            const auto& g2 = h->rbf2[(size_t)i * nk + jj];
            st.K = g1[0].K;
            st.Kp = rblock_padded_taps(ch, g1[0].K);
            for (int mth = 0; mth < 3; ++mth) {
                st.w1[mth] = (const uint4*)g1[mth].w_hi;
                st.w2[mth] = (const uint4*)g2[mth].w_hi;
                st.b1[mth] = g1[mth].bias;
                st.b2[mth] = g2[mth].bias;
                st.dil[mth] = g1[mth].dil;
            }
            rp.K = std::max(rp.K, st.K);
        }
        if (rp.wav && fuse_n == nk) rp.s_private = (int)std::min<size_t>(s_cap_bytes, (size_t)INT_MAX);
        rp.small_tile = DTTS_TUNE(h, 16384) ? 1 : 0;
        Timed tm(h, TV, s);
        LAUNCH(rblock_launch(rp, ch, s));
        return DTTS_OK;
    }

    int rb2x(int j) {
        const auto& fv = h->rbf1[(size_t)i * nk + j];
        RB2xParams rp;
        whole_rb_params(rp, j, j);
        rp.K = fv[0].K;
        rp.Kp = rblock_padded_taps(ch, fv[0].K);
        for (int m = 0; m < 2; ++m) {
            rp.w[m] = (const uint4*)fv[m].w_hi;
            rp.b[m] = fv[m].bias;
            rp.dil[m] = fv[m].dil;
        }
        Timed tm(h, TV, s);
        LAUNCH(rb2x_launch(rp, ch, s));
        return DTTS_OK;
    }

    int vpair(int j) {
        const auto& c1 = h->rb1[(size_t)i * nk + j];
        const auto& c2 = h->rb2[(size_t)i * nk + j];
        for (int mth = 0; mth < 3; ++mth)
            if (!vpair_pack_fits(c1[mth], ch, c1[0].K) || !vpair_pack_fits(c2[mth], ch, c1[0].K))
                return fail(h, DTTS_E_STATE, "resblock %d is not packed for vpair<%d>", i * nk + j, ch);
        const float* xin = Xf;
        for (int mth = 0; mth < 3; ++mth) {
            VPairParams vp;
            memset(&vp, 0, sizeof vp);
            vp.x = xin;
            vp.w1 = (const uint4*)c1[mth].w_hi;
            vp.w2 = (const uint4*)c2[mth].w_hi;
            vp.b1 = c1[mth].bias;
            vp.b2 = c2[mth].bias;
            vp.lens = lout;
            vp.B = B;
            vp.T = Tcur;
            vp.K = c1[mth].K;
            vp.dil = c1[mth].dil;
            vp.div = (float)nk;
            vp.slope = last_stage ? 0.01f : 0.1f;
            vp.el = el;
            vp.tile_ctr = n_ctr < N_CTR ? ctrs + n_ctr++ : nullptr;
            vp.ovf = (exact && h->guard_on) ? h->ovf_dev : nullptr;
            const bool s16 = exact && !DTTS_TUNE(h, 32768);
            vp.x16 = (s16 && mth > 0) ? 1 : 0;
            if (mth < 2) {
                vp.y = mth == 0 ? Rf : Rg;
                vp.mode = 1;
                vp.y16 = s16 ? 1 : 0;
            } else {
                vp.y = Sf;
                vp.mode = j == 0 ? 1 : (j == nk - 1 ? 3 : 2);
                vp.ya = exact ? nullptr : Sa;
                vp.drop_y = exact ? 0 : 1;
            }
            xin = vp.y;
            Timed tm(h, TV, s);
            LAUNCH(vpair_launch(vp, ch, s));
        }
        return DTTS_OK;
    }

    int convs(int j) {
        if (exact) return fail(h, DTTS_E_STATE, "DTTS_VOC_F16: resblock %d has no fused kernel", i * nk + j);
        const auto& c1 = h->rb1[(size_t)i * nk + j];
        if (c1[0].frag != 32) return fail(h, DTTS_E_STATE, "resblock %d is packed for vpair, not for the per-convolution kernels", i * nk + j);
        const int n = h->resblock2 ? 2 : 3;
        for (int mth = 0; mth < n; ++mth) {
            const bf* xa = mth == 0 ? Xa : Ra;
            if (!h->resblock2) {
                VConvParams p = vparams(c1[mth], xa, lout, B, Tcur);
                p.ya = Ta;
                p.ldya = ch;
                p.slope = 0.1f;
                Timed tm(h, TV, s);
                LAUNCH(vconv_launch(p, s));
                xa = Ta;
            }
            VConvParams p = vparams(h->resblock2 ? c1[mth] : h->rb2[(size_t)i * nk + j][mth], xa, lout, B, Tcur);
            p.res = mth == 0 ? Xf : Rf;
            p.ldres = ch;
            if (mth < n - 1) {
                p.yf = Rf;
                p.ldyf = ch;
                p.ya = Ra;
                p.ldya = ch;
                p.slope = 0.1f;
            } else {
                p.yf = Sf;
                p.ldyf = ch;
                if (j > 0) {
                    p.res2 = Sf;
                    p.ldres2 = ch;
                }
                if (j == nk - 1) {
                    p.div = (float)nk;
                    p.ya = Sa;
                    p.ldya = ch;
                    p.slope = last_stage ? 0.01f : 0.1f;
                }
            }
            Timed tm(h, TV, s);
            LAUNCH(vconv_launch(p, s));
        }
        return DTTS_OK;
    }
};

int hifigan_forward_fused(dtts_ctx* h, const float* mel, const int32_t* lens, int B, int T, float* wav, hipStream_t s) {
    const dtts_config& c = h->cfg;
    const bool exact = c.vocoder_precision == DTTS_VOC_F16;
    const int nup = c.n_upsamples, nk = c.n_resblock_kernels;
    const int melC = h->conv_pre.C_in_pad;
    const bool fuse = exact || !c.vocoder_unfused;
    const StageGeom g = stage_geom(c, B, T);
    const FusePlan plan = fuse_plan(h, g, B, fuse);
    const size_t max_elems = g.max_elems, s_elems = plan.s_elems;
    HIPCHK(h->a_voc.reserve((s_elems - max_elems) * sizeof(float) + max_elems * (4 * sizeof(float) + 4 * sizeof(bf)) + (size_t)B * T * melC * sizeof(bf) +
                            (size_t)(nup + 2) * B * sizeof(int) + (64 << 10), s));
    Arena& A = h->a_voc;
    VocRun r = {h, s, B, nk, exact, exact ? EL_F16 : EL_BF16, wav};
    r.s_cap_bytes = s_elems * sizeof(float);
    float* Xf = r.Xf = A.alloc<float>(max_elems);
    r.Rf = A.alloc<float>(max_elems);
    float* Sf = r.Sf = A.alloc<float>(s_elems);
    r.Rg = A.alloc<float>(max_elems);
    bf* Xa = r.Xa = A.alloc<bf>(max_elems);
    r.Ra = A.alloc<bf>(max_elems);
    r.Ta = A.alloc<bf>(max_elems);
    bf* Sa = r.Sa = A.alloc<bf>(max_elems);
    bf* melb = A.alloc<bf>((size_t)B * T * melC);
    int* lensS = A.alloc<int>((size_t)(nup + 1) * B);
    r.ctrs = A.alloc<unsigned>(N_CTR);
    if (!Xf || !r.Rf || !Sf || !r.Rg || !Xa || !r.Ra || !r.Ta || !Sa || !melb || !lensS || !r.ctrs) return fail(h, DTTS_E_NOMEM, "vocoder workspace");
    HIPCHK(hipMemsetAsync(r.ctrs, 0, N_CTR * sizeof(unsigned), s));
    scale_lens(c, lens, lensS, B, T, s);
    if (lens && (h->hop & 3) == 0 && ((uintptr_t)wav & 15) == 0) {
        const long long n = (long long)T * h->hop;
        hipLaunchKernelGGL(zero_wav_tails_kernel, dim3((unsigned)((n / 4 + 255) / 256), B), dim3(256), 0, s, wav, lens, T, h->hop);
        HIPCHK(hipGetLastError());
    } else if (lens) HIPCHK(hipMemsetAsync(wav, 0, (size_t)B * T * h->hop * sizeof(float), s));
    struct SpanGuard {
        dtts_ctx* h;
        Timed* t;
        ~SpanGuard() {
            h->voc_span = false;
            delete t;
        }
    } span{h, nullptr};
    if (h->timers[TV].enabled) {
        span.t = new Timed(h, TV, s);
        if (span.t->e1) h->timers[TV].launches -= 1;
        h->voc_span = true;
    }
    if (exact) {
        VConvParams p = vparams_x3(h->conv_pre, mel, c.audio_num_mel_bins, 1.f, lensS, B, T);
        p.yf = Sf;
        p.ldyf = g.ch[0];
        Timed tm(h, TV, s);
        LAUNCH(vconv_launch(p, s));
    } else {
        LAUNCH(f32_to_bf16_pad_launch(mel, melb, (long long)B * T, c.audio_num_mel_bins, melC, s));
        VConvParams p = vparams(h->conv_pre, melb, lensS, B, T);
        p.ya = Sa;
        p.ldya = g.ch[0];
        p.slope = 0.1f;
        Timed tm(h, TV, s);
        LAUNCH(vconv_launch(p, s));
    }
    for (int i = 0; i < nup; ++i) {
        const int u = c.upsample_rates[i], ch = g.ch[i + 1], Tin = (int)g.rows[i];
        const int* lin = lensS + (size_t)i * B;
        bool need_xa = false;
        for (int j = 0; j < nk; ++j) need_xa = need_xa || rb_path(h, fuse, ch, (size_t)i * nk + j) == RB_CONVS;
        {
            VConvParams p = exact ? vparams_x3(h->ups[i], Sf, 2 * ch, 0.1f, lin, B, Tin) : vparams(h->ups[i], Sa, lin, B, Tin);
            p.small_tiles = exact;
            p.yf = Xf;
            p.ldyf = u * ch;
            p.ya = need_xa ? Xa : nullptr;
            p.ldya = u * ch;
            p.slope = 0.1f;
            Timed tm(h, TV, s);
            LAUNCH(vconv_launch(p, s));
        }
        r.i = i;
        r.ch = ch;
        r.Tcur = (int)g.rows[i + 1];
        r.lout = lensS + (size_t)(i + 1) * B;
        r.last_stage = i == nup - 1;
        for (int j = 0; j < nk; ++j) {
            const RbPath path = rb_path(h, fuse, ch, (size_t)i * nk + j);
            const int rc = path == RB_WHOLE ? (h->resblock2 ? r.rb2x(j) : r.rblock(j, plan.fuse_n[i]))
                                            : (path == RB_VPAIR ? r.vpair(j) : r.convs(j));
            if (rc) return rc;
        }
    }
    if (!r.post_done) {
        const int Tcur = (int)g.rows[nup], ch = g.ch[nup];
        VConvParams p = exact ? vparams_x3(h->conv_post, Sf, ch, 0.01f, lensS + (size_t)nup * B, B, Tcur)
                              : vparams(h->conv_post, Sa, lensS + (size_t)nup * B, B, Tcur);
        p.yf = wav;
        p.ldyf = 1;
        p.post_tanh = 1;
        p.bad = h->bad_dev;
        Timed tm(h, TV, s);
        LAUNCH(vconv_launch(p, s));
    }
    return DTTS_OK;
}

int hifigan_forward_x3(dtts_ctx* h, const float* mel, const int32_t* lens, int B, int T, float* wav, hipStream_t s) {
    const dtts_config& c = h->cfg;
    const int nup = c.n_upsamples, nk = c.n_resblock_kernels;
    const size_t max_elems = stage_geom(c, B, T).max_elems;
    HIPCHK(h->a_voc.reserve(4 * (max_elems * sizeof(float) + 256) + (size_t)(nup + 2) * B * sizeof(int) + 8192, s));
    float* bufX = h->a_voc.alloc<float>(max_elems);
    float* bufR = h->a_voc.alloc<float>(max_elems);
    float* bufT = h->a_voc.alloc<float>(max_elems);
    float* bufS = h->a_voc.alloc<float>(max_elems);
    int* lensS = h->a_voc.alloc<int>((size_t)(nup + 1) * B);
    if (!bufX || !bufR || !bufT || !bufS || !lensS) return fail(h, DTTS_E_NOMEM, "vocoder workspace");
    scale_lens(c, lens, lensS, B, T, s);
    int Tcur = T, ch = c.upsample_initial_channel;
    {
        ConvParams p = base_params(mel, c.audio_num_mel_bins, B, T, T, bufS, ch);
        p.in_lens = lensS;
        p.out_lens = lensS;
        Timed tm(h, TV, s);
        LAUNCH(conv1d_launch(h->conv_pre, p, s));
    }
    for (int i = 0; i < nup; ++i) {
        const int u = c.upsample_rates[i];
        const int* lin = lensS + (size_t)i * B;
        const int* lout = lensS + (size_t)(i + 1) * B;
        ch /= 2;
        {
            ConvParams p = base_params(bufS, 2 * ch, B, Tcur, Tcur, bufX, u * ch);
            p.in_lens = lin;
            p.out_lens = lin;
            p.pre_act = 1;
            p.pre_slope = 0.1f;
            Timed tm(h, TV, s);
            LAUNCH(conv1d_launch(h->ups[i], p, s));
        }
        Tcur *= u;
        auto conv = [&](const PackedConv& L, const float* xin, const float* res, float* y, bool last, int j) -> int {
            ConvParams p = base_params(xin, ch, B, Tcur, Tcur, y, ch);
            p.in_lens = lout;
            p.out_lens = lout;
            p.pre_act = 1;
            p.pre_slope = 0.1f;
            if (res) set_res(p, 0, res, ch);
            if (last && j > 0) {
                p.seg[0].res2 = bufS;
                p.seg[0].ld_res2 = ch;
            }
            if (last && j == nk - 1) p.out_div = (float)nk;
            Timed tm(h, TV, s);
            LAUNCH(conv1d_launch(L, p, s));
            return DTTS_OK;
        };
        for (int j = 0; j < nk; ++j) {
            const auto& c1 = h->rb1[(size_t)i * nk + j];
            const int n = h->resblock2 ? 2 : 3;
            for (int mth = 0; mth < n; ++mth) {
                const float* xin = mth == 0 ? bufX : bufR;
                const bool last = mth == n - 1;
                if (!h->resblock2)
                    if (int rc = conv(c1[mth], xin, nullptr, bufT, false, j)) return rc;
                const PackedConv& L = h->resblock2 ? c1[mth] : h->rb2[(size_t)i * nk + j][mth];
                if (int rc = conv(L, h->resblock2 ? xin : bufT, xin, last ? bufS : bufR, last, j)) return rc;
            }
        }
    }
    {
        const int* lout = lensS + (size_t)nup * B;
        ConvParams p = base_params(bufS, ch, B, Tcur, Tcur, wav, 1);
        p.in_lens = lout;
        p.out_lens = lout;
        p.zero_masked = 1;
        p.pre_act = 1;
        p.pre_slope = 0.01f;
        p.post_act = 2;
        Timed tm(h, TV, s);
        LAUNCH(conv1d_launch(h->conv_post, p, s));
    }
    return DTTS_OK;
}

}

extern "C" {

int dtts_hifigan_hop(dtts_handle h) { return h ? h->hop : 0; }

int dtts_wav_to_int16(dtts_handle h, const float* wav, const int32_t* lens, int B, int T, int norm, int16_t* out, dtts_stream stream) {
    if (!h) return DTTS_E_INVAL;
    if (!h->vocoder_ready) return fail(h, DTTS_E_STATE, "vocoder weights not finalized");
    if (!wav || !out || B <= 0 || T <= 0) return fail(h, DTTS_E_INVAL, "dtts_wav_to_int16: bad argument");
    hipStream_t s = (hipStream_t)stream;
    if (!h->amax_bits || h->amax_cap < B) {
        if (h->amax_bits) {
            HIPCHK(hipDeviceSynchronize());
            (void)hipFree(h->amax_bits);
            h->amax_bits = nullptr;
        }
        HIPCHK(hipMalloc((void**)&h->amax_bits, sizeof(unsigned) * std::max(B, 256)));
        h->amax_cap = std::max(B, 256);
    }
    LAUNCH(wav_to_int16_launch(wav, lens, h->hop, B, (long long)T * h->hop, norm, h->amax_bits, out, s));
    return DTTS_OK;
}

int dtts_hifigan_forward(dtts_handle h, const float* mel, const int32_t* lens, int B, int T, float* wav, dtts_stream stream) {
    if (!h) return DTTS_E_INVAL;
    if (!h->vocoder_ready) return fail(h, DTTS_E_STATE, "vocoder weights not finalized");
    if (!mel || !wav || B <= 0 || T <= 0) return fail(h, DTTS_E_INVAL, "dtts_hifigan_forward: bad argument");
    hipStream_t s = (hipStream_t)stream;
    const dtts_config& c = h->cfg;
    Timed t_voc(h, DTTS_TIMER_STAGE_HIFIGAN, s);
    if (c.vocoder_precision != DTTS_VOC_BF16X3) {
        if (B > DTTS_MAX_VOCODER_BATCH) return fail(h, DTTS_E_INVAL, "dtts_hifigan_forward: B = %d exceeds %d utterances per call", B, DTTS_MAX_VOCODER_BATCH);
        if (c.vocoder_precision == DTTS_VOC_F16 && ((uintptr_t)mel & 15))
            return fail(h, DTTS_E_INVAL, "dtts_hifigan_forward: DTTS_VOC_F16 reads mel with 16-byte loads: the pointer must be 16-byte aligned");
        const int rc = hifigan_forward_fused(h, mel, lens, B, T, wav, s);
        if (rc == DTTS_OK && h->bad_dev && h->bad_host) HIPCHK(hipMemcpyAsync((void*)h->bad_host, h->bad_dev, sizeof(unsigned), hipMemcpyDeviceToHost, s));
        return rc;
    }
    return hifigan_forward_x3(h, mel, lens, B, T, wav, s);
}

int dtts_vocoder_range_guard(dtts_handle h, int enable) {
    if (!h) return DTTS_E_INVAL;
    if (enable && h->cfg.vocoder_precision != DTTS_VOC_F16) return fail(h, DTTS_E_INVAL, "the range guard exists for DTTS_VOC_F16 only (the other modes have fp32's exponent range)");
    h->guard_on = enable != 0;
    return DTTS_OK;
}

int dtts_vocoder_clamped(dtts_handle h, int64_t* count, int reset, dtts_stream stream) {
    if (!h || !count) return DTTS_E_INVAL;
    if (!h->ovf_dev) return fail(h, DTTS_E_STATE, "vocoder weights not finalized");
    unsigned long long v = 0;
    hipStream_t s = (hipStream_t)stream;
    HIPCHK(hipMemcpyAsync(&v, h->ovf_dev, sizeof v, hipMemcpyDeviceToHost, s));
    if (reset) HIPCHK(hipMemsetAsync(h->ovf_dev, 0, sizeof v, s));
    HIPCHK(hipStreamSynchronize(s));
    *count = (int64_t)v;
    return DTTS_OK;
}

int dtts_vocoder_nonfinite(dtts_handle h, int64_t* count) {
    if (!h || !count) return DTTS_E_INVAL;
    if (!h->vocoder_ready) return fail(h, DTTS_E_STATE, "vocoder weights not finalized");
    *count = h->bad_host ? (int64_t)*h->bad_host : 0;
    return DTTS_OK;
}

int dtts_vocoder_fp16_bound(dtts_handle h, float mel_abs_max, double* worst_case, double* rms_estimate) {
    if (!h || !(mel_abs_max >= 0.f)) return DTTS_E_INVAL;
    if (!h->vocoder_ready) return fail(h, DTTS_E_STATE, "vocoder weights not finalized");
    const bool f16 = h->cfg.vocoder_precision == DTTS_VOC_F16;
    if (worst_case) *worst_case = f16 ? h->wc_const + h->wc_lin * (double)mel_abs_max : 0.0;
    if (rms_estimate) *rms_estimate = f16 ? std::sqrt(h->est_const * h->est_const + h->est_lin * h->est_lin * (double)mel_abs_max * mel_abs_max) : 0.0;
    return DTTS_OK;
}

}
```

dict_tts_amd/hparams.py:

```python
import os

import yaml

hparams = {}


def _override(old, new):
    for k, v in new.items():
        if isinstance(v, dict) and isinstance(old.get(k), dict):
            _override(old[k], v)
        else:
            old[k] = v


def load_config_chain(config_fn, _seen=None):
    seen = set() if _seen is None else _seen
    if not os.path.exists(config_fn):
        return {}
    with open(config_fn) as f:
        cur = yaml.safe_load(f) or {}
    seen.add(config_fn)
    out = {}
    bases = cur.get("base_config", [])
    if not isinstance(bases, list):
        bases = [bases]
    for c in bases:
        if c.startswith("."):
            c = os.path.normpath(os.path.join(os.path.dirname(config_fn), c))
        if c not in seen:
            _override(out, load_config_chain(c, seen))
    _override(out, cur)
    return out


def apply_overrides(hp, hparams_str):
    if not hparams_str:
        return hp
    for item in hparams_str.split(","):
        k, v = item.split("=")
        v = v.strip("'\" ")
        node = hp
        for part in k.split(".")[:-1]:
            node = node[part]
        k = k.split(".")[-1]
        old = node.get(k)
        if v in ("True", "False") or isinstance(old, (bool, list, dict)):
            if isinstance(old, list):
                v = v.replace(" ", ",")
            node[k] = eval(v, {"__builtins__": {}}, {})
        elif old is None:
            node[k] = yaml.safe_load(v)
        else:
            node[k] = type(old)(v)
    return hp


def set_hparams(config="", exp_name="", hparams_str="", global_hparams=True, work_root="checkpoints"):
    hp = {}
    if config:
        hp.update(load_config_chain(config))
    work_dir = os.path.join(work_root, exp_name) if exp_name else ""
    if work_dir and os.path.exists(os.path.join(work_dir, "config.yaml")):
        with open(os.path.join(work_dir, "config.yaml")) as f:
            hp.update(yaml.safe_load(f) or {})
    hp["work_dir"] = work_dir
    apply_overrides(hp, hparams_str)
    hp["exp_name"] = exp_name
    hp["infer"] = True
    if global_hparams:
        hparams.clear()
        hparams.update(hp)
    return hp


BIAOBEI_DEFAULTS = {
    "hidden_size": 192, "num_heads": 2, "enc_ffn_kernel_size": 5, "word_size": 8000, "value_embedding_size": 185,
    "audio_num_mel_bins": 80, "latent_size": 16, "fvae_enc_dec_hidden": 192, "fvae_kernel_size": 5,
    "fvae_dec_n_layers": 4, "fvae_enc_n_layers": 8, "prior_glow_hidden": 64, "glow_kernel_size": 3,
    "prior_glow_n_blocks": 4, "dur_predictor_layers": 3, "dur_predictor_kernel": 5, "frames_multiple": 4,
    "language": "zh", "use_post_glow": False, "use_prior_glow": True, "dur_scale": "log", "dur_level": "word",
    "audio_sample_rate": 22050, "hop_size": 256, "use_spk_embed": False, "use_spk_id": False, "num_spk": 1,
    "vocoder": "dict_tts_amd.vocoder.HifiGAN", "vocoder_ckpt": "", "use_word_input": True, "use_dict": True,
}

HIFIGAN_V3 = {
    "resblock": "2", "upsample_rates": [8, 8, 4], "upsample_kernel_sizes": [16, 16, 8],
    "upsample_initial_channel": 256, "resblock_kernel_sizes": [3, 5, 7],
    "resblock_dilation_sizes": [[1, 2], [2, 6], [3, 12]],
}

HIFIGAN_DEFAULTS = {
    "resblock": "1", "upsample_rates": [8, 8, 2, 2], "upsample_kernel_sizes": [16, 16, 4, 4],
    "upsample_initial_channel": 512, "resblock_kernel_sizes": [3, 7, 11],
    "resblock_dilation_sizes": [[1, 3, 5], [1, 3, 5], [1, 3, 5]],
}


def speaker_kind(hp):
    hp = {**BIAOBEI_DEFAULTS, **(hp or {})}
    if not (hp.get("use_spk_embed") or hp.get("use_spk_id")):
        return None
    num_spk = int(hp.get("num_spk", 1) or 1)
    if num_spk <= 1:
        which = "use_spk_id" if hp.get("use_spk_id") else "use_spk_embed"
        raise ValueError(f"{which}=True needs num_spk > 1, but num_spk={num_spk}: the reference builds no spk_embed_proj then and fails in "
                         f"forward.  Override it with the checkpoint's speaker count, e.g. --hparams num_spk=N")
    return "id" if hp.get("use_spk_id") else "embed"


def fill_abi_config(cfg, hp=None, voc=None, n_phone=None, vocoder_precision=None):
    hp = {**BIAOBEI_DEFAULTS, **(hp or {})}
    if hp.get("use_post_glow"):
        raise NotImplementedError("use_post_glow=True is outside the Dict-TTS path (egs/egs_bases/tts/dict_tts.yaml:4)")
    speaker_kind(hp)
    if not hp.get("use_prior_glow", True) or hp.get("dur_scale", "log") != "log":
        raise NotImplementedError("only use_prior_glow=True / dur_scale=log are implemented")
    for k in ("hidden_size", "num_heads", "enc_ffn_kernel_size", "word_size", "value_embedding_size",
              "audio_num_mel_bins", "latent_size", "fvae_enc_dec_hidden", "fvae_kernel_size", "fvae_dec_n_layers",
              "fvae_enc_n_layers", "prior_glow_hidden", "glow_kernel_size", "prior_glow_n_blocks",
              "dur_predictor_layers", "dur_predictor_kernel", "frames_multiple"):
        setattr(cfg, k, int(hp[k]))
    cfg.language_zh = 1 if hp.get("language", "zh") == "zh" else 0
    if n_phone is not None:
        cfg.n_phone = int(n_phone)
    if voc is not None:
        resblock = str(voc.get("resblock", "1")).strip()
        if resblock not in ("1", "2"):
            raise NotImplementedError(f"resblock={voc.get('resblock')!r}: the generator's 'resblock' is '1' (ResBlock1) or '2' (ResBlock2)")
        n_dil = 3 if resblock == "1" else 2
        ur, uk = list(voc["upsample_rates"]), list(voc["upsample_kernel_sizes"])
        rk, rd = list(voc["resblock_kernel_sizes"]), [list(d) for d in voc["resblock_dilation_sizes"]]
        cfg.upsample_initial_channel = int(voc["upsample_initial_channel"])
        cfg.n_upsamples = len(ur)
        for i in range(len(ur)):
            cfg.upsample_rates[i] = int(ur[i])
            cfg.upsample_kernel_sizes[i] = int(uk[i])
        cfg.n_resblock_kernels = len(rk)
        for i in range(len(rk)):
            cfg.resblock_kernel_sizes[i] = int(rk[i])
            if len(rd[i]) != n_dil:
                raise NotImplementedError(f"resblock_dilation_sizes[{i}] = {rd[i]}: resblock '{resblock}' (ResBlock{resblock}) expects exactly "
                                          f"{n_dil} dilations per kernel size")
            if any(int(d) < 1 for d in rd[i]):
                raise ValueError(f"resblock_dilation_sizes[{i}] = {rd[i]}: dilations must be >= 1")
            for j in range(3):
                cfg.resblock_dilation_sizes[i][j] = int(rd[i][j]) if j < n_dil else 0
    if vocoder_precision is not None:
        cfg.vocoder_precision = int(vocoder_precision)
    cfg.tune_flags = int((hp or {}).get("dtts_tune_flags", 0)) | int((voc or {}).get("dtts_tune_flags", 0))
    cfg.debug_redzone = 1 if ((hp or {}).get("dtts_debug_redzone") or (voc or {}).get("dtts_debug_redzone")) else 0
    return cfg
```

Measured before the change: 1.307 million.

## Run C=64 fused ResBlock kernel on 16x16x32 MFMA shape

Makes the fused ResBlock kernel generic over the MFMA shape and selects 16x16x32 for 64-channel stages, which halves the k-step count and drops the tap padding those stages needed on 32x32x16 (via a half-group tail in rb_contract). Weights for those stages are packed in the matching fragment layout, and the launch checks that the packed fragment shape agrees with the kernel. A debug mode deliberately mismatches the shape to test that check. The MT=5 C=64 configuration loses its overflow-guard variant, so guarded f16 runs fall back to smaller tiles.

```diff
diff --git a/dict_tts_amd/csrc/context.hip b/dict_tts_amd/csrc/context.hip
--- a/dict_tts_amd/csrc/context.hip
+++ b/dict_tts_amd/csrc/context.hip
@@ -114,6 +114,7 @@
     (void)hipGetDevice(&h->device);
     if (hipDeviceGetAttribute(&h->n_cu, hipDeviceAttributeMultiprocessorCount, h->device) != hipSuccess || h->n_cu <= 0) h->n_cu = 256;
     h->debug_rz = cfg->debug_redzone != 0;
+    h->debug_misorder = cfg->debug_redzone == 2;
     h->a_fft.debug = h->a_enc.debug = h->a_dec.debug = h->a_voc.debug = h->a_spk.debug = h->a_post.debug = h->debug_rz;
     *out = h;
     return DTTS_OK;
diff --git a/dict_tts_amd/csrc/ctx.h b/dict_tts_amd/csrc/ctx.h
--- a/dict_tts_amd/csrc/ctx.h
+++ b/dict_tts_amd/csrc/ctx.h
@@ -157,6 +157,7 @@
     unsigned long long noise_seed = 0;
     unsigned long long* ovf_dev = nullptr;
     bool guard_on = false;
+    bool debug_misorder = false;
     unsigned* bad_dev = nullptr;
     volatile unsigned* bad_host = nullptr;
     double wc_lin = 0, wc_const = 0, est_lin = 0, est_const = 0;
diff --git a/dict_tts_amd/csrc/rb_common.h b/dict_tts_amd/csrc/rb_common.h
--- a/dict_tts_amd/csrc/rb_common.h
+++ b/dict_tts_amd/csrc/rb_common.h
@@ -108,6 +108,10 @@
 #pragma unroll
         for (int e = 0; e < 4; ++e) a[4 * qi + e] = v[e];
     }
+    static __device__ __forceinline__ void add_quad(acc_t& a, int qi, const f32x4& v) {
+#pragma unroll
+        for (int e = 0; e < 4; ++e) a[4 * qi + e] += v[e];
+    }
     template <int EL>
     static __device__ __forceinline__ void mma(acc_t& d, const uint4* w, const uint4* const (&x)[XF], const acc_t& c) {
         d = mfma16<EL>(w[0], *x[0], c);
@@ -132,6 +136,10 @@
     static __device__ __forceinline__ int xoff(int lane, int pitch) { return (lane & 15) * pitch + (lane >> 4) * 16; }
     static __device__ __forceinline__ f32x4 quad(const acc_t& a, int qi) { return a.q[qi]; }
     static __device__ __forceinline__ void set_quad(acc_t& a, int qi, const f32x4& v) { a.q[qi] = v; }
+    static __device__ __forceinline__ void add_quad(acc_t& a, int qi, const f32x4& v) {
+#pragma unroll
+        for (int e = 0; e < 4; ++e) a.q[qi][e] += v[e];
+    }
     template <int EL>
     static __device__ __forceinline__ void mma(acc_t& d, const uint4* w, const uint4* const (&x)[XF], const acc_t& c) {
 #pragma unroll
@@ -156,16 +164,17 @@
         for (int n = 0; n < NTW; ++n) ring[s][n] = w[(size_t)s * kg_stride + n * 64];
 }
 
-template <int EL, int MT, int NT, int NKG, int PITCH, bool CINIT, int MH = 1, class SH = MfmaShape<32>>
+template <int EL, int MT, int NT, int NKG, int PITCH, bool CINIT, int MH = 1, class SH = MfmaShape<32>, int NU = 4>
 __device__ __forceinline__ void rb_group(typename SH::acc_t (&acc)[MH * MT][NT], const typename SH::acc_t (&cinit)[NT], uint4 (&ring)[SH::RD][NT * SH::WF],
                                          uint4 (&xa)[MT], const char* act, const uint4* wpf, int xb, int dilP, int g) {
     constexpr int GPT = (NKG >= 4) ? NKG / 4 : 1;
     constexpr int KGS = NKG * SH::CI * 2 * SH::WF;
     constexpr int HSTRIDE = MT * 32 * PITCH;
     constexpr int RD = SH::RD, WF = SH::WF, KB = SH::KB;
-    static_assert(4 % RD == 0, "a group of 4 steps is whole turns of the ring");
-#pragma unroll
-    for (int u = 0; u < 4; ++u) {
+    static_assert(NU % RD == 0, "a group is whole turns of the ring");
+    static_assert(NU == 4 || (NKG < 4 && NU % NKG == 0), "a short group is whole taps");
+#pragma unroll
+    for (int u = 0; u < NU; ++u) {
 #pragma unroll
         for (int h = 0; h < MH; ++h) {
             if (h == 0) {
@@ -221,6 +230,8 @@
     constexpr int TU = (NKG >= 4) ? 1 : 4 / NKG;
     constexpr int GPT = (NKG >= 4) ? NKG / 4 : 1;
     constexpr int KGS = NKG * SH::CI * 2 * SH::WF;
+    constexpr bool TAIL = (NKG == 2 && SH::FRAG == 16);
+    const int SG = TAIL ? S - 2 : S;
     uint4 xa[MT];
 #pragma unroll
     for (int p = 0; p < MT; ++p) xa[p] = *(const uint4*)(act + xrow0 + (p / SH::XF * 32 + p % SH::XF * SH::XROWS) * PITCH);
@@ -248,7 +259,7 @@
                 for (int n = 0; n < NT; ++n) acc[m][n] = (*cinit)[n];
         }
     }
-    for (; s0 < S; s0 += 4) {
+    for (; s0 < SG; s0 += 4) {
         const acc_t(&dummy)[NT] = *(const acc_t(*)[NT])acc[0];
         rb_group<EL, MT, NT, NKG, PITCH, false, MH, SH>(acc, dummy, ring, xa, act, wpf, xb, dilP, g);
         wpf += 4 * KGS;
@@ -260,6 +271,10 @@
         } else {
             xb += TU * dilP;
         }
+    }
+    if constexpr (TAIL) {
+        const acc_t(&dummy)[NT] = *(const acc_t(*)[NT])acc[0];
+        rb_group<EL, MT, NT, NKG, PITCH, false, MH, SH, 2>(acc, dummy, ring, xa, act, wpf, xb, dilP, 0);
     }
 }
 
diff --git a/dict_tts_amd/csrc/rblock.h b/dict_tts_amd/csrc/rblock.h
--- a/dict_tts_amd/csrc/rblock.h
+++ b/dict_tts_amd/csrc/rblock.h
@@ -51,9 +51,11 @@
     return h;
 }
 
+constexpr int rblock_mfma_shape(int C) { return C == 64 ? 16 : 32; }
+
 bool rblock_supported(int C, int K);
 int rblock_padded_taps(int C, int K);
-hipError_t rblock_launch(const RBlockParams& p, int C, hipStream_t stream);
+hipError_t rblock_launch(const RBlockParams& p, int C, int frag, hipStream_t stream);
 long long rblock_private_rows(int C, int halo, int B, int T);
 int rblock_stage_tile_rows(int C, int halo);
 bool rblock_stage_launch_fits(int C, int halo, int B, bool wav);
diff --git a/dict_tts_amd/csrc/rblock.hip b/dict_tts_amd/csrc/rblock.hip
--- a/dict_tts_amd/csrc/rblock.hip
+++ b/dict_tts_amd/csrc/rblock.hip
@@ -22,14 +22,16 @@
 #define RB_T(k)
 #endif
 
-template <int C, int MT, int NT, int WT, int WC, int EL, int PS, bool GUARD, bool TB = false>
+template <int C, int MT, int NT, int WT, int WC, int EL, int PS, bool GUARD, bool TB = false, class SH = MfmaShape<32>>
 __global__ __launch_bounds__(64 * WT * WC, (64 * WT * WC <= 256) ? 2 : 1) void rblock_kernel(const RBlockParams p) {
     static_assert(WC * NT * 32 == C, "channel tiling must cover C");
+    static_assert(!TB || SH::FRAG == 32, "the two-buffer form was only ever built on 32x32x16");
+    typedef typename SH::acc_t acc_t;
     extern __shared__ __attribute__((aligned(16))) char smem[];
     constexpr int THREADS = 64 * WT * WC;
     constexpr int W = 32 * MT * WT;
     constexpr int PITCH = C * 2 + 16;
-    constexpr int NKG = C / 16;
+    constexpr int NKG = C / SH::CI;
     constexpr int EP = C * 4 + 16;
     constexpr int F4 = C / 4, SROWS = WT * 32;
     constexpr size_t ACT_BYTES = (size_t)(W + 2 * RB_GUARD) * PITCH;
@@ -84,17 +86,15 @@
         while (pre[bb + 1] <= jj) ++bb;
         bb = __builtin_amdgcn_readfirstlane(bb);
     };
-    auto load_x = [&](f32x16 (&d)[NT], int m, int bb, int base, int ln) {
+    auto load_x = [&](acc_t (&d)[NT], int m, int bb, int base, int ln) {
         const auto rs = __builtin_amdgcn_make_buffer_rsrc((void*)(p.x + (long long)bb * p.T * C), 0, ln * C * 4, 0x00020000);
-        const int o0 = ((base + wt * MT * 32 + (lane & 31)) * C + wc * NT * 32 + 4 * (lane >> 5)) * 4;
+        const int o0 = ((base + wt * MT * 32 + SH::row(lane, 0)) * C + wc * NT * 32 + SH::chan(lane, 0)) * 4;
 #pragma unroll
         for (int n = 0; n < NT; ++n)
 #pragma unroll
             for (int q = 0; q < 4; ++q) {
-                const u32x4 v = __builtin_amdgcn_raw_buffer_load_b128(rs, o0 + (m * 32 * C + n * 32 + 8 * q) * 4, 0, RB_X_AUX);
-                const f32x4 f = __builtin_bit_cast(f32x4, v);
-#pragma unroll
-                for (int e = 0; e < 4; ++e) d[n][4 * q + e] = f[e];
+                const u32x4 v = __builtin_amdgcn_raw_buffer_load_b128(rs, o0 + (m * 32 * C + n * 32 + SH::row(0, q) * C + SH::chan(0, q)) * 4, 0, RB_X_AUX);
+                SH::set_quad(d[n], q, __builtin_bit_cast(f32x4, v));
             }
     };
     auto len_of = [&](int bb) { return __builtin_amdgcn_readfirstlane(pre[2 * p.B + 1 + bb]); };
@@ -110,7 +110,7 @@
         t0 = blockIdx.x * TTo - (p.wav ? PH : 0);
         if (t0 + (p.wav ? PH : 0) >= len) return;
     }
-    f32x16 xr[MT][NT];
+    acc_t xr[MT][NT];
     if constexpr (PS) {
 #pragma unroll
         for (int m = 0; m < MT; ++m) load_x(xr[m], m, b, t0 - H, len);
@@ -131,15 +131,12 @@
 #pragma unroll
             for (int n = 0; n < NT; ++n)
 #pragma unroll
-                for (int q = 0; q < 4; ++q) {
-                    const f32x4 v = *(const f32x4*)(stage + (wt * 32 + (lane & 31)) * EP + ((wc * NT + n) * 32 + 8 * q + 4 * (lane >> 5)) * 4);
-#pragma unroll
-                    for (int e = 0; e < 4; ++e) xr[m][n][4 * q + e] = v[e];
-                }
-        }
-    }
-
-    const int kg_stride = (C / 32) * 64;
+                for (int q = 0; q < 4; ++q)
+                    SH::set_quad(xr[m][n], q, *(const f32x4*)(stage + (wt * 32 + SH::row(lane, q)) * EP + ((wc * NT + n) * 32 + SH::chan(lane, q)) * 4));
+        }
+    }
+
+    const int kg_stride = (C / 32) * SH::WF * 64;
     int r = 0;
 
 #ifdef RB_STAMP
@@ -155,13 +152,15 @@
         wt = wave % WT, wc = wave / WT;
         c4 = tid % F4, r0 = tid / F4;
     }
-    const int xlane = (RB_GUARD + wt * MT * 32 + (lane & 31)) * PITCH + (lane >> 5) * 16;
-    const size_t wlane = (size_t)(wc * NT) * 64 + lane;
+    const int xlane = (RB_GUARD + wt * MT * 32 + SH::row(lane, 0)) * PITCH + SH::chan(lane, 0) * 4;
+    const size_t wlane = (size_t)(wc * NT) * SH::WF * 64 + lane;
     if constexpr (PS) r = __builtin_amdgcn_readfirstlane(r);
     else r = 0;
     const RBlockParams::Set& R = p.rb[PS ? r : 0];
     const int Kr = R.K;
-    constexpr bool REAL_STEPS = (NKG < 4);
+    constexpr bool REAL_STEPS = (C == 32);
+    static_assert(!REAL_STEPS || SH::FRAG == 32, "rb2_contract is written for 32x32x16");
+    static_assert(REAL_STEPS || NKG >= 4 || (NKG == 2 && SH::FRAG == 16), "whole groups of four k-steps, or rb_contract's half group");
     const int S = (REAL_STEPS ? Kr : R.Kp) * NKG;
     const bool last_rb = !PS || r + 1 == p.nrb;
     const int mode = (!PS || p.nrb == 1 || r == 0) ? p.mode : (last_rb ? p.last_mode : 1);
@@ -195,70 +194,77 @@
     const auto rs_s = p.s_private ? __builtin_amdgcn_make_buffer_rsrc((void*)p.S, 0, p.s_private, 0x00020000)
                                   : __builtin_amdgcn_make_buffer_rsrc((void*)(p.S + brow * C), 0, len * C * 4, 0x00020000);
 
-    auto load_bias = [&](f32x4 (&bb)[NT][4], const float* bias) {
+    constexpr int NBQ = 4 / SH::QB;
+    auto load_bias = [&](f32x4 (&bb)[NT][NBQ], const float* bias) {
 #pragma unroll
         for (int n = 0; n < NT; ++n)
 #pragma unroll
-            for (int q = 0; q < 4; ++q) bb[n][q] = *(const f32x4*)(bias + (wc * NT + n) * 32 + 8 * q + 4 * (lane >> 5));
+            for (int q = 0; q < NBQ; ++q) bb[n][q] = *(const f32x4*)(bias + (wc * NT + n) * 32 + SH::chan(lane, q * SH::QB));
     };
     const bool all_inb = base_t >= 0 && base_t + W <= len;
     int n_ovf = 0;
-    auto write_act_impl = [&](char* dst, const f32x16 (&v)[MT][NT], auto masked_tag) {
+    auto write_act_impl = [&](char* dst, const acc_t (&v)[MT][NT], auto masked_tag) {
         constexpr bool MASKED = decltype(masked_tag)::value;
+        int ln = lane;
+        if constexpr (SH::FRAG == 16) asm volatile("" : "+v"(ln));
 #pragma unroll
         for (int m = 0; m < MT; ++m) {
-            const int row = (wt * MT + m) * 32 + (lane & 31);
-            const int t = base_t + row;
-            const bool inb = !MASKED || (t >= 0 && t < len);
-            const bool counted = inb && row >= H && row < H + TT;
+            int row[SH::QB];
+            bool inb[SH::QB], counted[SH::QB];
+#pragma unroll
+            for (int rh = 0; rh < SH::QB; ++rh) {
+                row[rh] = (wt * MT + m) * 32 + SH::row(ln, rh);
+                const int t = base_t + row[rh];
+                inb[rh] = !MASKED || (t >= 0 && t < len);
+                counted[rh] = inb[rh] && row[rh] >= H && row[rh] < H + TT;
+            }
 #pragma unroll
             for (int n = 0; n < NT; ++n)
 #pragma unroll
                 for (int q = 0; q < 4; ++q) {
-                    const int co = (wc * NT + n) * 32 + 8 * q + 4 * (lane >> 5);
-                    f32x4 v4 = {v[m][n][4 * q], v[m][n][4 * q + 1], v[m][n][4 * q + 2], v[m][n][4 * q + 3]};
+                    constexpr int QBM = SH::QB - 1;
+                    const int co = (wc * NT + n) * 32 + SH::chan(ln, q);
+                    const f32x4 v4 = SH::quad(v[m][n], q);
                     uint2 pk = act4<EL>(v4, 0.1f);
-                    if constexpr (GUARD) n_ovf += counted ? ovf4(v4, 0.1f) : 0;
+                    if constexpr (GUARD) n_ovf += counted[q & QBM] ? ovf4(v4, 0.1f) : 0;
                     if constexpr (MASKED) {
-                        if (!inb) pk = make_uint2(0, 0);
+                        if (!inb[q & QBM]) pk = make_uint2(0, 0);
                     }
-                    *(uint2*)(dst + (RB_GUARD + row) * PITCH + co * 2) = pk;
+                    *(uint2*)(dst + (RB_GUARD + row[q & QBM]) * PITCH + co * 2) = pk;
                 }
         }
     };
-    auto write_act = [&](char* dst, const f32x16 (&v)[MT][NT]) {
+    auto write_act = [&](char* dst, const acc_t (&v)[MT][NT]) {
         if (all_inb) write_act_impl(dst, v, std::false_type{});
         else write_act_impl(dst, v, std::true_type{});
     };
 
-    uint4 ring[4][NT];
-    f32x4 bb[NT][4];
+    uint4 ring[SH::RD][NT * SH::WF];
+    f32x4 bb[NT][NBQ];
     RB_T(10);
-    rb_preload<NT>(ring, R.w1[0] + wlane, kg_stride);
+    rb_preload(ring, R.w1[0] + wlane, kg_stride);
     load_bias(bb, R.b1[0]);
     write_act(act, xr);
     RB_T(0);
     __syncthreads();
     RB_T(1);
 
-    f32x16 acc[MT][NT];
+    acc_t acc[MT][NT];
 #pragma unroll 1
     for (int it = 0; it < 3; ++it) {
-        f32x16 cinit[NT];
+        acc_t cinit[NT];
 #pragma unroll
         for (int n = 0; n < NT; ++n)
 #pragma unroll
-            for (int q = 0; q < 4; ++q)
-#pragma unroll
-                for (int e = 0; e < 4; ++e) cinit[n][4 * q + e] = bb[n][q][e];
+            for (int q = 0; q < 4; ++q) SH::set_quad(cinit[n], q, bb[n][q / SH::QB]);
         load_bias(bb, R.b2[it]);
         const int d = R.dil[it];
         if constexpr (REAL_STEPS) {
             if (S) rb2_contract<EL, MT, NT, NKG, PITCH, 4, true>(acc, ring, act, xlane - ((Kr - 1) / 2) * d * PITCH, R.w1[it] + wlane, S, d * PITCH, cinit);
             else rb_contract<EL, MT, NT, NKG, PITCH, true, 1>(acc, ring, act, 0, R.w1[it] + wlane, 0, 0, &cinit);
         } else
-            rb_contract<EL, MT, NT, NKG, PITCH, true, 1>(acc, ring, act, xlane - ((Kr - 1) / 2) * d * PITCH, R.w1[it] + wlane, S, d * PITCH, &cinit);
-        rb_preload<NT>(ring, R.w2[it] + wlane, kg_stride);
+            rb_contract<EL, MT, NT, NKG, PITCH, true, 1, SH>(acc, ring, act, xlane - ((Kr - 1) / 2) * d * PITCH, R.w1[it] + wlane, S, d * PITCH, &cinit);
+        rb_preload(ring, R.w2[it] + wlane, kg_stride);
         RB_T(2);
         if constexpr (!TB) __syncthreads();
         RB_T(3);
@@ -271,15 +277,13 @@
 #pragma unroll
             for (int n = 0; n < NT; ++n)
 #pragma unroll
-                for (int q = 0; q < 4; ++q)
-#pragma unroll
-                    for (int e = 0; e < 4; ++e) xr[m][n][4 * q + e] += bb[n][q][e];
+                for (int q = 0; q < 4; ++q) SH::add_quad(xr[m][n], q, bb[n][q / SH::QB]);
         if (it < 2) load_bias(bb, R.b1[it + 1]);
         if constexpr (REAL_STEPS) {
             if (S) rb2_contract<EL, MT, NT, NKG, PITCH, 4, false>(xr, ring, act2, xlane - ((Kr - 1) / 2) * PITCH, R.w2[it] + wlane, S, PITCH, cinit);
         } else
-            rb_contract<EL, MT, NT, NKG, PITCH, false, 1>(xr, ring, act2, xlane - ((Kr - 1) / 2) * PITCH, R.w2[it] + wlane, S, PITCH);
-        if (it < 2) rb_preload<NT>(ring, R.w1[it + 1] + wlane, kg_stride);
+            rb_contract<EL, MT, NT, NKG, PITCH, false, 1, SH>(xr, ring, act2, xlane - ((Kr - 1) / 2) * PITCH, R.w2[it] + wlane, S, PITCH);
+        if (it < 2) rb_preload(ring, R.w1[it + 1] + wlane, kg_stride);
         if (PS && p.tile_ctr && last_rb && it == 2 && tid == 0) pre[3 * p.B + 1] = G + (int)claim;
         RB_T(6);
         if (!TB || it == 2) __syncthreads();
@@ -329,12 +333,7 @@
 #pragma unroll
         for (int n = 0; n < NT; ++n)
 #pragma unroll
-            for (int q = 0; q < 4; ++q) {
-                f32x4 v;
-#pragma unroll
-                for (int e = 0; e < 4; ++e) v[e] = xr[m][n][4 * q + e];
-                *(f32x4*)(stg + (lane & 31) * EP + (n * 32 + 8 * q + 4 * (lane >> 5)) * 4) = v;
-            }
+            for (int q = 0; q < 4; ++q) *(f32x4*)(stg + SH::row(lane, q) * EP + (n * 32 + SH::chan(lane, q)) * 4) = SH::quad(xr[m][n], q);
         if (has_next) load_x(xr[m], m, bn, t0n - H, lenn);
         __builtin_amdgcn_fence(__ATOMIC_RELEASE, "wavefront");
         __builtin_amdgcn_wave_barrier();
@@ -472,7 +471,10 @@
 
 template <int C, int MT, int NT, int WT, int WC, int EL, int PS, bool GUARD = false, bool TB = false>
 static hipError_t rb_launch_cfg(const RBlockParams& p, hipStream_t stream) {
+    typedef MfmaShape<rblock_mfma_shape(C)> SH;
     constexpr int W = 32 * MT * WT;
+    for (int j = 0; j < p.nrb; ++j)
+        if (!(p.rb[j].K & 1) || p.rb[j].Kp != rblock_padded_taps(C, p.rb[j].K)) return hipErrorInvalidValue;
     const int H = rblock_halo(p), TT = W - 2 * H;
     if (TT < 32) return hipErrorInvalidValue;
     if ((long long)p.T * C * 4 >= (1LL << 31)) return hipErrorInvalidValue;
@@ -483,10 +485,12 @@
     q.pre_off = (int)lds;
     if (PS) lds += rb_table_bytes(p.B);
     if (lds > 160 * 1024) return hipErrorOutOfMemory;
-    if constexpr (EL == EL_F16 && !GUARD) {
+    constexpr bool HAS_GUARD = !(C == 64 && MT == 5);
+    if constexpr (EL == EL_F16 && !GUARD && HAS_GUARD) {
         if (p.ovf) return rb_launch_cfg<C, MT, NT, WT, WC, EL, PS, true, TB>(p, stream);
     }
-    auto kern = rblock_kernel<C, MT, NT, WT, WC, EL, PS, GUARD, TB>;
+    if (EL == EL_F16 && !HAS_GUARD && p.ovf) return hipErrorInvalidValue;
+    auto kern = rblock_kernel<C, MT, NT, WT, WC, EL, PS, GUARD, TB, SH>;
     static bool configured_dev[64] = {};
     int cur_dev = 0;
     (void)hipGetDevice(&cur_dev);
@@ -540,7 +544,9 @@
 }
 
 int rblock_padded_taps(int C, int K) {
-    const int nkg = C / 16;
+    const int sh = rblock_mfma_shape(C);
+    const int nkg = C / (sh == 16 ? 32 : 16);
+    if (sh == 16 && nkg == 2) return K;
     int kp = K;
     while ((kp * nkg) % 4) ++kp;
     return kp;
@@ -576,7 +582,7 @@
     if (C == 128 && few(256)) return rb_launch_cfg<128, 4, 1, 1, 4, EL, 1>(p, stream);
     if (C == 256 && few(128)) return rb_launch_cfg<256, 2, 1, 1, 8, EL, 1>(p, stream);
     if (C == 32) return rb_launch_cfg<32, 4, 1, 4, 1, EL, 0>(p, stream);
-    if (C == 64 && p.K >= 7 && !p.small_tile) RB_TRY((rb_launch_cfg<64, 5, 1, 4, 2, EL, 1>(p, stream)));
+    if (C == 64 && p.K >= 7 && !p.small_tile && !(EL == EL_F16 && p.ovf)) RB_TRY((rb_launch_cfg<64, 5, 1, 4, 2, EL, 1>(p, stream)));
     if (C == 64) RB_TRY((rb_launch_cfg<64, 4, 1, 4, 2, EL, 1>(p, stream)));
     if (C == 64) return rb_launch_cfg<64, 4, 1, 2, 2, EL, 1>(p, stream);
     if (C == 128) RB_TRY((rb_launch_cfg<128, 4, 1, 2, 4, EL, 1>(p, stream)));
@@ -587,7 +593,9 @@
     return hipErrorInvalidValue;
 }
 
-hipError_t rblock_launch(const RBlockParams& p, int C, hipStream_t stream) {
+hipError_t rblock_launch(const RBlockParams& p, int C, int frag, hipStream_t stream) {
+    if (C != 32 && C != 64 && C != 128 && C != 256) return hipErrorInvalidValue;
+    if (frag != rblock_mfma_shape(C)) return hipErrorInvalidValue;
     return p.el == EL_F16 ? rb_launch_el<EL_F16>(p, C, stream) : rb_launch_el<EL_BF16>(p, C, stream);
 }
 
diff --git a/dict_tts_amd/csrc/vocoder.hip b/dict_tts_amd/csrc/vocoder.hip
--- a/dict_tts_amd/csrc/vocoder.hip
+++ b/dict_tts_amd/csrc/vocoder.hip
@@ -115,14 +115,14 @@
     return true;
 }
 
-bool pack_rb_fused(dtts_ctx* h, Need& need, PackedConv& L, int eng, const std::string& base, int ch, int k, int dil) {
+bool pack_rb_fused(dtts_ctx* h, Need& need, PackedConv& L, int eng, const std::string& base, int ch, int k, int dil, int frag) {
     const HostTensor* w = folded_weight(h, need, base);
     std::vector<float> bias = bias_of(need, base);
     if (!w || bias.empty()) return false;
     const float* pw = w->f.data();
     const int slack = ch >= 64 ? 1 : 2;
     const bool ok = pack_conv(h, L, eng, ch, ch, rblock_padded_taps(ch, k) + slack,
-                              [=](int co, int ci, int tap) { return tap < k ? pw[((size_t)co * ch + ci) * k + tap] : 0.f; }, bias, dil, 1, 0);
+                              [=](int co, int ci, int tap) { return tap < k ? pw[((size_t)co * ch + ci) * k + tap] : 0.f; }, bias, dil, 1, 0, 0, -1, frag);
     L.K = k;
     return ok;
 }
@@ -212,7 +212,7 @@
         h->rbf1[i].resize(2);
         for (int mth = 0; ok && mth < 2; ++mth)
             ok = pack_rb_fused(h, need, h->rbf1[i][mth], eng_rb, v + "resblocks." + std::to_string(i) + ".convs." + std::to_string(mth), ch, k,
-                               c.resblock_dilation_sizes[j][mth]);
+                               c.resblock_dilation_sizes[j][mth], 32);
     }
     for (int i = 0; ok && !rb2x && eng_rb != ENG_BF16X3 && i < c.n_upsamples * nk; ++i) {
         const int j = i % nk, k = c.resblock_kernel_sizes[j];
@@ -227,8 +227,8 @@
         h->rbf2[i].resize(3);
         const std::string r = v + "resblocks." + std::to_string(i);
         for (int mth = 0; ok && mth < 3; ++mth) {
-            ok = pack_rb_fused(h, need, h->rbf1[i][mth], eng_rb, r + ".convs1." + std::to_string(mth), ch, k, c.resblock_dilation_sizes[j][mth]);
-            ok = ok && pack_rb_fused(h, need, h->rbf2[i][mth], eng_rb, r + ".convs2." + std::to_string(mth), ch, k, 1);
+            ok = pack_rb_fused(h, need, h->rbf1[i][mth], eng_rb, r + ".convs1." + std::to_string(mth), ch, k, c.resblock_dilation_sizes[j][mth], rblock_mfma_shape(ch));
+            ok = ok && pack_rb_fused(h, need, h->rbf2[i][mth], eng_rb, r + ".convs2." + std::to_string(mth), ch, k, 1, rblock_mfma_shape(ch));
         }
     }
     ok = ok && pack_plain(h, need, h->conv_post, eng, v + "conv_post", 1, 1, 3);
@@ -417,12 +417,16 @@
         whole_rb_params(rp, j, j_last);
         rp.nrb = j_last - j + 1;
         rp.last_mode = j_last == nk - 1 ? 2 : 1;
+        int frag = 0;
         for (int jj = j; jj <= j_last; ++jj) {
             RBlockParams::Set& st = rp.rb[jj - j];
             const auto& g1 = h->rbf1[(size_t)i * nk + jj];
             const auto& g2 = h->rbf2[(size_t)i * nk + jj];
             st.K = g1[0].K;
             st.Kp = rblock_padded_taps(ch, g1[0].K);
+            if (jj == j) frag = g1[0].frag;
+            for (int mth = 0; mth < 3; ++mth)
+                if (g1[mth].frag != frag || g2[mth].frag != frag) frag = 0;
             for (int mth = 0; mth < 3; ++mth) {
                 st.w1[mth] = (const uint4*)g1[mth].w_hi;
                 st.w2[mth] = (const uint4*)g2[mth].w_hi;
@@ -434,8 +438,9 @@
         }
         if (rp.wav && fuse_n == nk) rp.s_private = (int)std::min<size_t>(s_cap_bytes, (size_t)INT_MAX);
         rp.small_tile = DTTS_TUNE(h, 16384) ? 1 : 0;
+        if (h->debug_misorder) frag = frag == 16 ? 32 : 16;
         Timed tm(h, TV, s);
-        LAUNCH(rblock_launch(rp, ch, s));
+        LAUNCH(rblock_launch(rp, ch, frag, s));
         return DTTS_OK;
     }
 
diff --git a/dict_tts_amd/hparams.py b/dict_tts_amd/hparams.py
--- a/dict_tts_amd/hparams.py
+++ b/dict_tts_amd/hparams.py
@@ -148,5 +148,6 @@
     if vocoder_precision is not None:
         cfg.vocoder_precision = int(vocoder_precision)
     cfg.tune_flags = int((hp or {}).get("dtts_tune_flags", 0)) | int((voc or {}).get("dtts_tune_flags", 0))
-    cfg.debug_redzone = 1 if ((hp or {}).get("dtts_debug_redzone") or (voc or {}).get("dtts_debug_redzone")) else 0
+    rz = (hp or {}).get("dtts_debug_redzone") or (voc or {}).get("dtts_debug_redzone")
+    cfg.debug_redzone = (2 if rz is not True and rz == 2 else 1) if rz else 0
     return cfg
```

New measurement: 1.323 million, median of 6. 1.01x the previous value.
